# TomasDelaney/A-Deep-Reinforcement-Learning-Enabled-Soft-Exoskeleton-for-Parkinson-s-Patients

Measured on AMD Instinct MI355X. Metric: env steps/sec (batched exo sim) + TD7 grad-steps/sec at 1/2/4/8 MI355X, higher is better.
Workload: dtype f64 sim + bf16 TD7

## Files before the change

### a-deep-reinforcement-learning-enabled-soft-exoskeleton-for-parkinson-s-patients_amd/csrc/td7_fused.h

```cpp
#pragma once
#include <hip/hip_runtime.h>

#include <cstdint>

#include "exo_amd.h"
#include "philox.h"

namespace td7f {

typedef float floatx4 __attribute__((ext_vector_type(4)));
typedef __bf16 bf16x8 __attribute__((ext_vector_type(8)));
typedef _Float16 halfx8 __attribute__((ext_vector_type(8)));
typedef uint32_t u32x4 __attribute__((ext_vector_type(4)));
typedef uint32_t u32x2 __attribute__((ext_vector_type(2)));

template <typename T>
__device__ __forceinline__ T ldg(const T *p) {
    return *(const __attribute__((address_space(1))) T *)p;
}
template <typename T>
__device__ __forceinline__ void stg(T *p, T v) {
    *(__attribute__((address_space(1))) T *)p = v;
}

constexpr int NW = 4;
constexpr int NKG = 2;
constexpr int NTH = 64 * NW * NKG;
constexpr int PD = TD7F_PD;
constexpr int TR = 16;

enum Prec : int { PREC_BF16 = 1, PREC_F16 = 2, PREC_F32 = 3 };
enum Act : int { ACT_NONE = 0, ACT_RELU = 1, ACT_ELU = 2, ACT_TANH = 3 };

template <int P> struct Ty;
struct Ty16 {
    using E = uint16_t;
    static constexpr int EB = 2, KD = 32, SUB = 1;
};
template <> struct Ty<PREC_BF16> : Ty16 {
    static __device__ __forceinline__ floatx4 mfma(u32x4 a, u32x4 b, floatx4 c, int = 0) {
        return __builtin_amdgcn_mfma_f32_16x16x32_bf16(__builtin_bit_cast(bf16x8, a), __builtin_bit_cast(bf16x8, b),
                                                       c, 0, 0, 0);
    }
    static __device__ __forceinline__ uint16_t bits(float v) { return __builtin_bit_cast(uint16_t, (__bf16)v); }
    static __device__ __forceinline__ float val(uint16_t b) { return (float)__builtin_bit_cast(__bf16, b); }
    static constexpr float gs = 1.f;
};
template <> struct Ty<PREC_F16> : Ty16 {
    static __device__ __forceinline__ floatx4 mfma(u32x4 a, u32x4 b, floatx4 c, int = 0) {
        return __builtin_amdgcn_mfma_f32_16x16x32_f16(__builtin_bit_cast(halfx8, a), __builtin_bit_cast(halfx8, b), c,
                                                      0, 0, 0);
    }
    static __device__ __forceinline__ uint16_t bits(float v) { return __builtin_bit_cast(uint16_t, (_Float16)v); }
    static __device__ __forceinline__ float val(uint16_t b) { return (float)__builtin_bit_cast(_Float16, b); }
    static constexpr float gs = 1024.f;
};
template <> struct Ty<PREC_F32> {
    using E = float;
    static constexpr int EB = 4, KD = 16, SUB = 4;
    static __device__ __forceinline__ floatx4 mfma(u32x4 a, u32x4 b, floatx4 c, int j) {
        const floatx4 af = __builtin_bit_cast(floatx4, a), bf = __builtin_bit_cast(floatx4, b);
        return __builtin_amdgcn_mfma_f32_16x16x4f32(af[j], bf[j], c, 0, 0, 0);
    }
    static __device__ __forceinline__ float bits(float v) { return v; }
    static __device__ __forceinline__ float val(float b) { return b; }
    static constexpr float gs = 1.f;
};

__device__ __forceinline__ float act_fwd(int act, float x) {
    if (act == ACT_RELU) return x > 0.f ? x : 0.f;
    if (act == ACT_ELU) return x > 0.f ? x : __expf(x) - 1.0f;
    if (act == ACT_TANH) return tanhf(x);
    return x;
}
__device__ __forceinline__ float act_grad(int act, float y) {
    if (act == ACT_RELU) return y > 0.f ? 1.f : 0.f;
    if (act == ACT_ELU) return y > 0.f ? 1.f : y + 1.f;
    if (act == ACT_TANH) return 1.f - y * y;
    return 1.f;
}

struct Lin {
    const u32x4 *wf, *wb;
    const float *b;
    int N, K, ksf, ksb;
    const float *w;
    long ldw;
};

struct GDesc {
    const u32x4 *wp;
    int ks;
    int t0;
};

__device__ __forceinline__ void kgroup_range(int ks, int kg, int &kb, int &ke) {
    const int kA = ks >= 2 * PD ? ((ks / 2 + PD - 1) / PD) * PD : ks;
    kb = kg ? kA : 0;
    ke = kg ? ks : kA;
}

template <int TH>
__device__ __forceinline__ void ring_fill(u32x4 (&R)[PD][TH], const GDesc &g) {
    const int wv = threadIdx.x >> 6, w = wv % NW, kg = wv / NW, lane = threadIdx.x & 63;
    int kb, ke;
    kgroup_range(g.ks, kg, kb, ke);
    const bool live = ke > kb;
#pragma unroll
    for (int p = 0; p < PD; ++p)
#pragma unroll
        for (int i = 0; i < TH; ++i) {
            R[p][i] = ldg(g.wp + (live ? ((size_t)(g.t0 + w + NW * i) * g.ks + kb + p) * 64 : 0) + lane);
            __builtin_amdgcn_sched_barrier(0);
        }
}

struct EpiSrc {
    const float *p;
    long ld;
    int c0, row0, nrows, ncols;
};
template <int RT, int TH>
__device__ __forceinline__ void epi_prefetch(const EpiSrc &e, int t0, floatx4 (&ep)[RT][TH]) {
#pragma unroll
    for (int i = 0; i < TH; ++i) {
        const int wv = threadIdx.x >> 6;
        const int col = 16 * (t0 + wv % NW + NW * i) + 4 * ((threadIdx.x & 63) >> 4) - e.c0;
        const bool mine = (i < (TH + 1) / 2) == (wv < NW);
#pragma unroll
        for (int r = 0; r < RT; ++r) {
            const int row = (threadIdx.x & 15) + TR * r;
            const bool ok = e.p && mine && col >= 0 && col < e.ncols && (e.ld == 0 || e.row0 + row < e.nrows);
            ep[r][i] = ok ? ldg((const floatx4 *)(e.p + (e.ld ? (long)(e.row0 + row) * e.ld : 0) + col))
                          : floatx4{0.f, 0.f, 0.f, 0.f};
        }
    }
}

template <int P, int RT, int TH>
__device__ __forceinline__ void gemm(char *lds, int a_off, int lda, const GDesc &g, u32x4 (&R)[PD][TH],
                                     floatx4 (&acc)[RT][TH], const GDesc *next, const EpiSrc &es,
                                     floatx4 (&ep)[RT][TH]) {
    const int wv = threadIdx.x >> 6, w = wv % NW, kg = wv / NW, lane = threadIdx.x & 63;
    int kb, ke, nb = 0, ne = 0;
    kgroup_range(g.ks, kg, kb, ke);
    if (next) kgroup_range(next->ks, kg, nb, ne);
    epi_prefetch(es, g.t0, ep);
#pragma unroll
    for (int r = 0; r < RT; ++r)
#pragma unroll
        for (int i = 0; i < TH; ++i) acc[r][i] = floatx4{0.f, 0.f, 0.f, 0.f};
    if (ke > kb) {
        const u32x4 *bp[TH];
#pragma unroll
        for (int i = 0; i < TH; ++i) bp[i] = g.wp + ((size_t)(g.t0 + w + NW * i) * g.ks + kb) * 64 + lane;
        const char *ap = lds + a_off + ((lane & 15) * lda + 8 * (lane >> 4) + 32 * kb) * 2;
        const int n = ke - kb;
        u32x4 an[RT];
#pragma unroll
        for (int r = 0; r < RT; ++r) an[r] = *(const u32x4 *)(ap + r * TR * lda * 2);
        int s0 = 0;
        for (; s0 + PD < n; s0 += PD) {
#pragma unroll
            for (int p = 0; p < PD; ++p) {
                const int s = s0 + p;
                u32x4 x[RT];
#pragma unroll
                for (int r = 0; r < RT; ++r) {
                    x[r] = an[r];
                    an[r] = *(const u32x4 *)(ap + (r * TR * lda + 32 * (s + 1)) * 2);
                }
#pragma unroll
                for (int j = 0; j < Ty<P>::SUB; ++j)
#pragma unroll
                    for (int i = 0; i < TH; ++i) {
#pragma unroll
                        for (int r = 0; r < RT; ++r) acc[r][i] = Ty<P>::mfma(R[p][i], x[r], acc[r][i], j);
                        __builtin_amdgcn_sched_barrier(0);
                    }
#pragma unroll
                for (int i = 0; i < TH; ++i) {
                    R[p][i] = ldg(bp[i] + (s + PD) * 64);
                    __builtin_amdgcn_sched_barrier(0);
                }
            }
        }
        const u32x4 *np[TH];
        if (ne > nb)
#pragma unroll
            for (int i = 0; i < TH; ++i) np[i] = next->wp + ((size_t)(next->t0 + w + NW * i) * next->ks + nb) * 64 + lane;
#pragma unroll
        for (int p = 0; p < PD; ++p) {
            const int s = s0 + p;
            u32x4 x[RT];
#pragma unroll
            for (int r = 0; r < RT; ++r) {
                x[r] = an[r];
                if (p + 1 < PD) an[r] = *(const u32x4 *)(ap + (r * TR * lda + 32 * (s + 1)) * 2);
            }
#pragma unroll
            for (int j = 0; j < Ty<P>::SUB; ++j)
#pragma unroll
                for (int i = 0; i < TH; ++i) {
#pragma unroll
                    for (int r = 0; r < RT; ++r) acc[r][i] = Ty<P>::mfma(R[p][i], x[r], acc[r][i], j);
                    __builtin_amdgcn_sched_barrier(0);
                }
            if (ne > nb) {
#pragma unroll
                for (int i = 0; i < TH; ++i) {
                    R[p][i] = ldg(np[i] + p * 64);
                    __builtin_amdgcn_sched_barrier(0);
                }
            }
        }
    } else if (next) {
        ring_fill(R, *next);
    }
    constexpr int h = (TH + 1) / 2;
    floatx4 *red = (floatx4 *)lds + ((w * 64 + lane) * RT) * TH;
#pragma unroll
    for (int r = 0; r < RT; ++r)
#pragma unroll
        for (int i = 0; i < TH; ++i)
            if ((i < h) != (kg == 0)) red[r * TH + i] = acc[r][i];
    __syncthreads();
#pragma unroll
    for (int r = 0; r < RT; ++r)
#pragma unroll
        for (int i = 0; i < TH; ++i)
            if ((i < h) == (kg == 0)) acc[r][i] += red[r * TH + i];
}

constexpr int red_bytes(int rt, int tpw) { return NW * 64 * rt * tpw * 16; }

template <int TH>
__device__ __forceinline__ bool owns(int i) {
    return (i < (TH + 1) / 2) == ((threadIdx.x >> 6) < NW);
}
__device__ __forceinline__ int acc_col(int t0, int i) {
    const int wv = threadIdx.x >> 6;
    return 16 * (t0 + wv % NW + NW * i) + 4 * ((threadIdx.x & 63) >> 4);
}
__device__ __forceinline__ int acc_row(int r) { return (threadIdx.x & 15) + TR * r; }

struct R16 {
    int off, ld;
};
struct R32 {
    int off, ld;
};
constexpr R16 NO16{-1, 0};
constexpr R32 NO32{-1, 0};
__device__ __forceinline__ uint16_t *p16(char *lds, R16 r, int row, int col) {
    return (uint16_t *)(lds + r.off) + row * r.ld + col;
}
__device__ __forceinline__ float *p32(char *lds, R32 r, int row, int col) {
    return (float *)(lds + r.off) + row * r.ld + col;
}
template <int P>
__device__ __forceinline__ u32x2 pack4(const float (&v)[4]) {
    return u32x2{(uint32_t)Ty<P>::bits(v[0]) | ((uint32_t)Ty<P>::bits(v[1]) << 16),
                 (uint32_t)Ty<P>::bits(v[2]) | ((uint32_t)Ty<P>::bits(v[3]) << 16)};
}
template <int P>
__device__ __forceinline__ typename Ty<P>::E *pe(char *lds, R16 r, int row, int col) {
    return (typename Ty<P>::E *)(lds + r.off + row * r.ld * 2) + col;
}
template <int P>
__device__ __forceinline__ void put4(char *lds, R16 r, int row, int col, const float (&v)[4]) {
    if constexpr (Ty<P>::EB == 4) *(floatx4 *)pe<P>(lds, r, row, col) = floatx4{v[0], v[1], v[2], v[3]};
    else *(u32x2 *)pe<P>(lds, r, row, col) = pack4<P>(v);
}

template <int P, int RT, int TH>
__device__ __forceinline__ void epi_fwd(char *lds, const floatx4 (&acc)[RT][TH], const floatx4 (&bias)[RT][TH], int N,
                                        int act, R16 o16, int col0, R32 o32, float *g, long gld, int row0,
                                        int nrows) {
#pragma unroll
    for (int i = 0; i < TH; ++i) {
        if (!owns<TH>(i)) continue;
        const int n = acc_col(0, i);
        if (n >= N) continue;
        const floatx4 b = bias[0][i];
#pragma unroll
        for (int r = 0; r < RT; ++r) {
            const int row = acc_row(r);
            float v[4];
#pragma unroll
            for (int e = 0; e < 4; ++e) v[e] = act_fwd(act, acc[r][i][e] + b[e]);
            if (o16.off >= 0) put4<P>(lds, o16, row, col0 + n, v);
            if (o32.off >= 0) *(floatx4 *)p32(lds, o32, row, n) = floatx4{v[0], v[1], v[2], v[3]};
            if (g && row0 + row < nrows) stg((floatx4 *)(g + (long)(row0 + row) * gld + n), floatx4{v[0], v[1], v[2], v[3]});
        }
    }
}

template <int P, int RT, int TH>
__device__ __forceinline__ void epi_bwd(char *lds, const floatx4 (&acc)[RT][TH], int t0, int c0, int c1, int act,
                                        const floatx4 (&yv_)[RT][TH], R32 o32, float *g, long gld, R16 o16,
                                        float *part, int row0, int nrows) {
#pragma unroll
    for (int i = 0; i < TH; ++i) {
        if (!owns<TH>(i)) continue;
        const int col = acc_col(t0, i);
        const bool in = col >= c0 && col < c1;
        const int m = col - c0;
        float cs[4] = {0.f, 0.f, 0.f, 0.f};
#pragma unroll
        for (int r = 0; r < RT; ++r) {
            const int row = acc_row(r);
            const bool live = in && row0 + row < nrows;
            float v[4];
#pragma unroll
            for (int e = 0; e < 4; ++e) v[e] = live ? acc[r][i][e] * (1.f / Ty<P>::gs) : 0.f;
            if (live && act != ACT_NONE) {
                const floatx4 yv = yv_[r][i];
#pragma unroll
                for (int e = 0; e < 4; ++e) v[e] *= act_grad(act, yv[e]);
            }
#pragma unroll
            for (int e = 0; e < 4; ++e) cs[e] += v[e];
            if (in) {
                if (o32.off >= 0) *(floatx4 *)p32(lds, o32, row, m) = floatx4{v[0], v[1], v[2], v[3]};
                if (o16.off >= 0) {
                    float s[4] = {v[0] * Ty<P>::gs, v[1] * Ty<P>::gs, v[2] * Ty<P>::gs, v[3] * Ty<P>::gs};
                    put4<P>(lds, o16, row, m, s);
                }
                if (g && row0 + row < nrows) stg((floatx4 *)(g + (long)(row0 + row) * gld + m), floatx4{v[0], v[1], v[2], v[3]});
            }
        }
        if (part) {
#pragma unroll
            for (int e = 0; e < 4; ++e)
#pragma unroll
                for (int o = 1; o < 16; o <<= 1) cs[e] += __shfl_xor(cs[e], o, 64);
            if (in && (threadIdx.x & 15) == 0) stg((floatx4 *)(part + m), floatx4{cs[0], cs[1], cs[2], cs[3]});
        }
    }
}

template <int P, int NC>
__device__ __forceinline__ void thin(char *lds, R16 in, int xc0, int K, R32 wl, int ncols, R32 out, float scale) {
    constexpr int KS = NTH / TR;
    const int row = threadIdx.x / KS, sl = threadIdx.x % KS;
    float acc[NC];
#pragma unroll
    for (int j = 0; j < NC; ++j) acc[j] = 0.f;
#pragma unroll 2
    for (int k = sl; k < K; k += KS) {
        const float x = Ty<P>::val(*pe<P>(lds, in, row, xc0 + k));
#pragma unroll
        for (int j = 0; j < NC; ++j) acc[j] += x * *p32(lds, wl, j, k);
    }
#pragma unroll
    for (int j = 0; j < NC; ++j) {
#pragma unroll
        for (int o = KS / 2; o > 0; o >>= 1) acc[j] += __shfl_xor(acc[j], o, 64);
    }
    if (sl == 0)
#pragma unroll
        for (int j = 0; j < NC; ++j)
            if (j < ncols) *p32(lds, out, row, j) = acc[j] * scale;
}
constexpr int THIN_NC = 8;

template <int P>
__device__ __forceinline__ void make_dp(char *lds, R32 dy, int N, int act, const float *y, long yld, R16 o16,
                                        float *part, int row0, int nrows) {
    for (int n = threadIdx.x; n < N; n += NTH) {
        float cs = 0.f;
        for (int r = 0; r < TR; ++r) {
            float v = *p32(lds, dy, r, n);
            if (row0 + r >= nrows) v = 0.f;
            else if (act != ACT_NONE) v *= act_grad(act, ldg(y + (long)(row0 + r) * yld + n));
            *p32(lds, dy, r, n) = v;
            *pe<P>(lds, o16, r, n) = Ty<P>::bits(v * Ty<P>::gs);
            cs += v;
        }
        if (part) stg(part + n, cs);
    }
}

__device__ __forceinline__ void store_rows16(char *lds, R16 src, int col0, uint16_t *dst, long dld, int ncols,
                                             int rows, int row0, int nrows) {
    if (ncols % 8 == 0 && dld % 8 == 0 && col0 % 8 == 0 && src.ld % 8 == 0) {
        const int nq = ncols / 8;
        for (int k = threadIdx.x; k < rows * nq; k += NTH) {
            const int row = k / nq, c = 8 * (k - row * nq);
            if (row0 + row < nrows) stg((u32x4 *)(dst + (long)(row0 + row) * dld + c), *(const u32x4 *)p16(lds, src, row, col0 + c));
        }
        return;
    }
    for (int k = threadIdx.x; k < rows * ncols; k += NTH) {
        const int row = k / ncols, c = k - row * ncols;
        if (row0 + row < nrows) stg(dst + (long)(row0 + row) * dld + c, *p16(lds, src, row, col0 + c));
    }
}

struct RowStage {
    float v[TR];
};
__device__ __forceinline__ void row_issue(RowStage &s, const float *src, long sld, int ncols, int row0, int nrows) {
    const int c = min((int)threadIdx.x, ncols - 1);
#pragma unroll
    for (int r = 0; r < TR; ++r) s.v[r] = ldg(src + (long)(row0 + r < nrows ? row0 + r : row0) * sld + c);
}
__device__ __forceinline__ void row_add(RowStage &s, const RowStage &o) {
#pragma unroll
    for (int r = 0; r < TR; ++r) s.v[r] += o.v[r];
}
template <int P>
__device__ __forceinline__ void row_put16(char *lds, const RowStage &s, R16 dst, int col0, int ncols, int row0,
                                          int nrows, float scale = 1.f) {
    if ((int)threadIdx.x < ncols)
#pragma unroll
        for (int r = 0; r < TR; ++r)
            *pe<P>(lds, dst, r, col0 + threadIdx.x) = Ty<P>::bits(row0 + r < nrows ? s.v[r] * scale : 0.f);
}
__device__ __forceinline__ void row_put32(char *lds, const RowStage &s, R32 dst, int ncols, int row0, int nrows) {
    if ((int)threadIdx.x < ncols)
#pragma unroll
        for (int r = 0; r < TR; ++r) *p32(lds, dst, r, threadIdx.x) = row0 + r < nrows ? s.v[r] : 0.f;
}
struct Row16Stage {
    uint32_t v[TR];
};
__device__ __forceinline__ void row16_issue(Row16Stage &s, const uint16_t *src, long sld, int ncols, int row0,
                                            int nrows) {
    const int c = 2 * min((int)threadIdx.x, (ncols - 1) / 2);
#pragma unroll
    for (int r = 0; r < TR; ++r)
        s.v[r] = ldg((const uint32_t *)(src + (long)(row0 + r < nrows ? row0 + r : row0) * sld + c));
}
__device__ __forceinline__ void row16_put(char *lds, const Row16Stage &s, R16 dst, int col0, int ncols, int row0,
                                          int nrows) {
    const int c = 2 * threadIdx.x;
    if (c < ncols)
#pragma unroll
        for (int r = 0; r < TR; ++r) {
            const uint32_t v = row0 + r < nrows ? s.v[r] : 0u;
            *p16(lds, dst, r, col0 + c) = (uint16_t)(v & 0xffffu);
            if (c + 1 < ncols) *p16(lds, dst, r, col0 + c + 1) = (uint16_t)(v >> 16);
        }
}
template <int NC>
struct ThinStage {
    float v[NC];
};
template <int NC>
__device__ __forceinline__ void thin_issue(ThinStage<NC> &s, const float *W, long ldw, int j0, bool trans, int ncols,
                                           int K) {
    const int k = min((int)threadIdx.x, K - 1);
#pragma unroll
    for (int j = 0; j < NC; ++j) {
        const int jj = min(j, ncols - 1);
        s.v[j] = ldg(trans ? W + (long)k * ldw + j0 + jj : W + (long)(j0 + jj) * ldw + k);
    }
}
template <int P, int NC>
__device__ __forceinline__ void thin_put(char *lds, const ThinStage<NC> &s, R32 wl, int ncols, int K) {
    if ((int)threadIdx.x < K)
#pragma unroll
        for (int j = 0; j < NC; ++j) *p32(lds, wl, j, threadIdx.x) = j < ncols ? Ty<P>::val(Ty<P>::bits(s.v[j])) : 0.f;
}

__device__ __forceinline__ uint16_t *blk8(uint16_t *base, long ld, int c, int r) {
    return base + ((long)(c >> 4) * (ld >> 5) + (r >> 5)) * 512 + ((c & 15) + 16 * ((r & 31) >> 3)) * 8;
}
__device__ __forceinline__ float *blk4(float *base, long ld, int c, int r) {
    return base + ((long)(c >> 4) * (ld >> 4) + (r >> 4)) * 256 + ((c & 15) + 16 * ((r & 15) >> 2)) * 4;
}

template <int P>
__device__ __forceinline__ void save_xt(char *lds, R16 src, int col0, int ncols, void *xt_, long ld, int rows,
                                        int row0) {
    if constexpr (P == PREC_F32) {
        float *xt = (float *)xt_;
        for (int k = threadIdx.x; k < ncols * (rows / TR); k += NTH) {
            const int c = k % ncols, rb = (k / ncols) * TR;
            float v[TR];
#pragma unroll
            for (int j = 0; j < TR; ++j) v[j] = *pe<P>(lds, src, rb + j, col0 + c);
#pragma unroll
            for (int q = 0; q < 4; ++q)
                stg((floatx4 *)blk4(xt, ld, c, row0 + rb + 4 * q), floatx4{v[4 * q], v[4 * q + 1], v[4 * q + 2], v[4 * q + 3]});
        }
        return;
    }
    uint16_t *xt = (uint16_t *)xt_;
    if (col0 % 2 == 0 && src.ld % 2 == 0) {
        for (int k = threadIdx.x; k < ((ncols + 1) / 2) * (rows / TR); k += NTH) {
            const int c = 2 * (k % ((ncols + 1) / 2)), rb = (k / ((ncols + 1) / 2)) * TR;
            uint32_t lo[8], hi[8];
#pragma unroll
            for (int j = 0; j < 8; ++j) {
                const uint32_t r0 = *(const uint32_t *)p16(lds, src, rb + 2 * j, col0 + c);
                const uint32_t r1 = *(const uint32_t *)p16(lds, src, rb + 2 * j + 1, col0 + c);
                lo[j] = (r0 & 0xffffu) | (r1 << 16);
                hi[j] = (r0 >> 16) | (r1 & 0xffff0000u);
            }
            stg((u32x4 *)blk8(xt, ld, c, row0 + rb), u32x4{lo[0], lo[1], lo[2], lo[3]});
            stg((u32x4 *)blk8(xt, ld, c, row0 + rb + 8), u32x4{lo[4], lo[5], lo[6], lo[7]});
            if (c + 1 < ncols) {
                stg((u32x4 *)blk8(xt, ld, c + 1, row0 + rb), u32x4{hi[0], hi[1], hi[2], hi[3]});
                stg((u32x4 *)blk8(xt, ld, c + 1, row0 + rb + 8), u32x4{hi[4], hi[5], hi[6], hi[7]});
            }
        }
        return;
    }
    for (int k = threadIdx.x; k < ncols * (rows / TR); k += NTH) {
        const int c = k % ncols, rb = (k / ncols) * TR;
        uint32_t v[8];
#pragma unroll
        for (int j = 0; j < 8; ++j)
            v[j] = (uint32_t)*p16(lds, src, rb + 2 * j, col0 + c) |
                   ((uint32_t)*p16(lds, src, rb + 2 * j + 1, col0 + c) << 16);
        stg((u32x4 *)blk8(xt, ld, c, row0 + rb), u32x4{v[0], v[1], v[2], v[3]});
        stg((u32x4 *)blk8(xt, ld, c, row0 + rb + 8), u32x4{v[4], v[5], v[6], v[7]});
    }
}

template <int P>
__device__ __forceinline__ void norm_fwd(char *lds, R32 h, int N, int rows, float eps, R16 o16, int col0, R16 o16b,
                                         int col0b, R32 o32, float *g, long gld, float *mean_lds, float *gmean,
                                         int row0, int nrows) {
    const int tpr = NTH / rows;
    const int row = threadIdx.x / tpr, j0 = threadIdx.x % tpr;
    float acc = 0.f;
    for (int n = j0; n < N; n += tpr) acc += fabsf(*p32(lds, h, row, n));
    for (int o = tpr / 2; o > 0; o >>= 1) acc += __shfl_xor(acc, o, 64);
    const float m = acc / N, s = fmaxf(m, eps);
    for (int n = j0; n < N; n += tpr) {
        const float v = *p32(lds, h, row, n) / s;
        const auto b = Ty<P>::bits(v);
        if (o16.off >= 0) *pe<P>(lds, o16, row, col0 + n) = b;
        if (o16b.off >= 0) *pe<P>(lds, o16b, row, col0b + n) = b;
        if (o32.off >= 0) *p32(lds, o32, row, n) = v;
        if (g && row0 + row < nrows) stg(g + (long)(row0 + row) * gld + n, v);
    }
    if (j0 == 0) {
        if (mean_lds) mean_lds[row] = m;
        if (gmean && row0 + row < nrows) stg(gmean + row0 + row, m);
    }
}

template <int P>
__device__ __forceinline__ void norm_bwd(char *lds, R32 dy, R32 h, const float *mean, int N, float eps, float *dot,
                                         R16 o16, void *dpt, long dpt_ld, float *part, int row0, int nrows) {
    {
        constexpr int tpr = NTH / TR;
        const int row = threadIdx.x / tpr, j0 = threadIdx.x % tpr;
        float acc = 0.f;
        for (int n = j0; n < N; n += tpr) acc += *p32(lds, dy, row, n) * *p32(lds, h, row, n);
        for (int o = tpr / 2; o > 0; o >>= 1) acc += __shfl_xor(acc, o, 64);
        if (j0 == 0) dot[row] = acc;
    }
    __syncthreads();
    for (int n = threadIdx.x; n < N; n += NTH) {
        float csum = 0.f;
        uint32_t v[8];
        float f[TR];
#pragma unroll
        for (int r = 0; r < TR; ++r) {
            const float m = mean[r];
            float gx;
            if (m >= eps) {
                const float inv = 1.0f / m, c = dot[r] * inv * inv / N;
                const float xv = *p32(lds, h, r, n);
                const float sg = (xv > 0.f) ? 1.f : ((xv < 0.f) ? -1.f : 0.f);
                gx = *p32(lds, dy, r, n) * inv - sg * c;
            } else {
                gx = *p32(lds, dy, r, n) / eps;
            }
            if (row0 + r >= nrows) gx = 0.f;
            csum += gx;
            const auto hb = Ty<P>::bits(gx * Ty<P>::gs);
            *pe<P>(lds, o16, r, n) = hb;
            if constexpr (P == PREC_F32) {
                f[r] = hb;
            } else {
                if (r & 1) v[r >> 1] |= (uint32_t)hb << 16;
                else v[r >> 1] = hb;
            }
        }
        if (dpt) {
            if constexpr (P == PREC_F32) {
#pragma unroll
                for (int q = 0; q < 4; ++q)
                    stg((floatx4 *)blk4((float *)dpt, dpt_ld, n, row0 + 4 * q), floatx4{f[4 * q], f[4 * q + 1], f[4 * q + 2], f[4 * q + 3]});
            } else {
                stg((u32x4 *)blk8((uint16_t *)dpt, dpt_ld, n, row0), u32x4{v[0], v[1], v[2], v[3]});
                stg((u32x4 *)blk8((uint16_t *)dpt, dpt_ld, n, row0 + 8), u32x4{v[4], v[5], v[6], v[7]});
            }
        }
        if (part) stg(part + n, csum);
    }
}

struct Noise {
    uint64_t seed;
    uint32_t tag;
    unsigned long long *counter;
    uint32_t *ticket;
    float *sigma;
    float sigma_dec, clip, scale;
    const float *z;
    const int32_t *dec_count;
};

#ifdef EXO_STAMPS
static __device__ unsigned long long *g_td7f_stamps;
#define FSTAMP(si)                                                                                 \
    do {                                                                                           \
        unsigned long long _t;                                                                     \
        __builtin_amdgcn_sched_barrier(0);                                                         \
        asm volatile("s_memtime %0\n\ts_waitcnt lgkmcnt(0)" : "=s"(_t)::"memory");                \
        __builtin_amdgcn_sched_barrier(0);                                                         \
        if (g_td7f_stamps && threadIdx.x == 0 && (si) < 64)                                        \
            stg(g_td7f_stamps + (size_t)(blockIdx.x + blockIdx.y * gridDim.x) * 64 + (si), _t);    \
        ++(si);                                                                                    \
    } while (0)
#else
#define FSTAMP(si) do {} while (0)
#endif


template <int P, int RT, int TH>
__device__ __forceinline__ void layer_fwd(char *lds, u32x4 (&R)[PD][TH], R16 a, const Lin &L, const GDesc *next,
                                          int act, R16 o16, int col0, R32 o32, float *g, long gld, int row0,
                                          int nrows, int &si) {
    FSTAMP(si);
    floatx4 acc[RT][TH], bias[RT][TH];
    const GDesc gd{L.wf, L.ksf, 0};
    gemm<P, RT, TH>(lds, a.off, a.ld, gd, R, acc, next, EpiSrc{L.b, 0, 0, 0, 0, L.N}, bias);
    FSTAMP(si);
    epi_fwd<P, RT, TH>(lds, acc, bias, L.N, act, o16, col0, o32, g, gld, row0, nrows);
    __syncthreads();
}
template <int P, int RT, int TH>
__device__ __forceinline__ void layer_fwd(char *lds, u32x4 (&R)[PD][TH], R16 a, const Lin &L, const Lin *next, int act,
                                          R16 o16, int col0, R32 o32, float *g, long gld, int row0, int nrows,
                                          int &si) {
    GDesc gn{nullptr, 0, 0};
    if (next) gn = GDesc{next->wf, next->ksf, 0};
    layer_fwd<P, RT, TH>(lds, R, a, L, next ? &gn : (const GDesc *)nullptr, act, o16, col0, o32, g, gld, row0, nrows,
                         si);
}

template <int P, int NC>
__device__ __forceinline__ void layer_thin_fwd(char *lds, R16 a, const Lin &L, R32 wl, int act, R32 out, int rows,
                                               float *g, long gld, int row0, int nrows, int &si) {
    FSTAMP(si);
    thin<P, NC>(lds, a, 0, L.K, wl, L.N, out, 1.f);
    __syncthreads();
    for (int k = threadIdx.x; k < rows * L.N; k += NTH) {
        const int row = k / L.N, n = k - row * L.N;
        const float v = act_fwd(act, *p32(lds, out, row, n) + ldg(L.b + n));
        *p32(lds, out, row, n) = v;
        if (g && row0 + row < nrows) stg(g + (long)(row0 + row) * gld + n, v);
    }
    __syncthreads();
}

__device__ __forceinline__ void zero_lds(char *lds, int bytes) {
    for (int i = threadIdx.x * 16; i < bytes; i += NTH * 16) *(u32x4 *)(lds + i) = u32x4{0u, 0u, 0u, 0u};
}

template <int P>
__device__ __forceinline__ void noise_rows(char *lds, R32 a, int A, int rows, int row0, int nrows, const Noise &nz,
                                           float *out, R16 o1, int c1, R16 o2, int c2, bool ticket = true) {
    const float sg = ldg(nz.sigma);
    const unsigned long long call = ldg(nz.counter);
    for (int k = threadIdx.x; k < rows * A; k += NTH) {
        const int row = k / A, c = k - row * A;
        float v = 0.f;
        if (row0 + row < nrows) {
            const uint32_t i = (uint32_t)((row0 + row) * A + c);
            float z;
            if (nz.z) {
                z = ldg(nz.z + i);
            } else {
                uint32_t r[4];
                philox_block(nz.seed, nz.tag, call, i >> 1, r);
                float z0, z1;
                box_muller(r, z0, z1);
                z = (i & 1) ? z1 : z0;
            }
            float e = z * sg;
            if (nz.clip > 0.f) e = fminf(fmaxf(e, -nz.clip), nz.clip);
            v = fminf(fmaxf(*p32(lds, a, row, c) + e, -1.0f), 1.0f) * nz.scale;
            if (out) stg(out + i, v);
        }
        const auto b = Ty<P>::bits(v);
        if (o1.off >= 0) *pe<P>(lds, o1, row, c1 + c) = b;
        if (o2.off >= 0) *pe<P>(lds, o2, row, c2 + c) = b;
    }
    __syncthreads();
    if (ticket && threadIdx.x == 0) {
        __threadfence();
        if (atomicAdd(nz.ticket, 1u) == gridDim.x * gridDim.y - 1) {
            *nz.sigma = sg - (nz.dec_count ? nz.sigma_dec * (float)*nz.dec_count : nz.sigma_dec);
            if (!nz.z) *nz.counter = call + 1ull;
            *nz.ticket = 0u;
        }
    }
}

inline int round_up(int x, int m) { return (x + m - 1) / m * m; }
inline int kd_of(int prec) { return prec == PREC_F32 ? 16 : 32; }
inline int ks_of(int k, int kd = 32) { return round_up((k + kd - 1) / kd, PD); }
inline int ld16(int n, int kd = 32) { return ks_of(n, kd) * 32 + 16; }

struct Bump {
    int off;
    explicit Bump(int rt) : off(red_bytes(rt, 5)) {}
    R16 r16(int rows, int ld) {
        R16 r{off, ld};
        off += round_up(rows * ld * 2, 16);
        return r;
    }
    R32 r32(int rows, int ld) {
        R32 r{off, ld};
        off += round_up(rows * ld * 4, 16);
        return r;
    }
};

inline Lin lin_of(const td7f_lin &l) {
    return Lin{(const u32x4 *)l.wf, (const u32x4 *)l.wb, l.b, l.n_out, l.n_in, l.ksf, l.ksb, l.w, (long)l.ldw};
}
inline Noise noise_of(const td7f_noise &n) {
    return Noise{n.seed, n.tag, n.counter, n.ticket, n.sigma, n.sigma_dec, n.clip, n.scale, n.z, n.dec_count};
}

inline int th_of(const td7f_lin *ls, int n) {
    int th = 0;
    for (int i = 0; i < n; ++i) {
        if (!ls[i].wf || ls[i].ksf <= 0 || ls[i].ksf % PD || !ls[i].b) return -1;
        if (ls[i].n_out <= 16) {
            if (!ls[i].w || ls[i].ldw < ls[i].n_in) return -1;
            continue;
        }
        if (ls[i].n_out % 4) return -1;
        const int t = round_up((ls[i].n_out + 15) / 16, NW) / NW;
        if (th && t != th) return -1;
        th = t;
    }
    return th ? th : 4;
}

constexpr int LDS_MAX = 160 * 1024;

extern thread_local bool td7f_probe_mode;

template <typename K, typename A>
int launch(K kernel, dim3 grid, int lds, A args, hipStream_t st) {
    if (lds > LDS_MAX) return EXO_EINVAL;
    if (td7f_probe_mode) return EXO_OK;
    if (hipFuncSetAttribute((const void *)kernel, hipFuncAttributeMaxDynamicSharedMemorySize, lds) != hipSuccess)
        return EXO_EDEVICE;
    hipLaunchKernelGGL(kernel, grid, dim3(NTH), lds, st, args);
    return hipGetLastError() == hipSuccess ? EXO_OK : EXO_EDEVICE;
}

#define DISPATCH(PREC, TH, KERNEL, ...)                                                                 \
    ((PREC) == PREC_BF16  ? ((TH) == 5 ? launch(KERNEL<PREC_BF16, 5>, __VA_ARGS__)                      \
                                       : launch(KERNEL<PREC_BF16, 4>, __VA_ARGS__))                     \
     : (PREC) == PREC_F16 ? ((TH) == 5 ? launch(KERNEL<PREC_F16, 5>, __VA_ARGS__)                       \
                                       : launch(KERNEL<PREC_F16, 4>, __VA_ARGS__))                      \
                          : ((TH) == 5 ? launch(KERNEL<PREC_F32, 5>, __VA_ARGS__)                       \
                                       : launch(KERNEL<PREC_F32, 4>, __VA_ARGS__)))

}
```

### a-deep-reinforcement-learning-enabled-soft-exoskeleton-for-parkinson-s-patients_amd/csrc/td7_fused.hip

```cpp
#include "td7_fused.h"

#include <algorithm>
#include <cstdlib>

#include "adam_math.h"
#include "philox.h"

namespace td7f {

struct PackJob {
    const float *w;
    long ld;
    int N, K;
    u32x4 *wf, *wb;
    int ksf, ntf, ksb, ntb;
};
struct PackArgs {
    int njobs;
    long start[TD7F_MAX_PACK + 1];
    PackJob j[TD7F_MAX_PACK];
};

template <int P>
__device__ __forceinline__ float w_at(const PackJob &J, int n, int c) {
    const bool ok = n < J.N && c < J.K;
    const float x = ldg(J.w + (long)(ok ? n : 0) * J.ld + (ok ? c : 0));
    return ok ? x : 0.f;
}
__device__ __forceinline__ void pack_item_f32(const PackJob &J, long k, long nf, bool vec) {
    const int l = (int)(k & 63);
    float x[4];
    u32x4 *dst;
    if (k < nf) {
        const long blk = k >> 6;
        const int t = (int)(blk / J.ksf), s = (int)(blk % J.ksf);
        const int n = 16 * t + (l & 15), k0 = 16 * s + 4 * (l >> 4);
        if (vec && n < J.N && k0 + 4 <= J.K) {
            const floatx4 a0 = ldg((const floatx4 *)(J.w + (long)n * J.ld + k0));
            x[0] = a0[0], x[1] = a0[1], x[2] = a0[2], x[3] = a0[3];
        } else {
#pragma unroll
            for (int j = 0; j < 4; ++j) x[j] = w_at<PREC_F32>(J, n, k0 + j);
        }
        dst = J.wf + k;
    } else {
        const long blk = (k - nf) >> 6;
        const int t = (int)(blk / J.ksb), s = (int)(blk % J.ksb);
        const int c = 16 * t + (l & 15), n0 = 16 * s + 4 * (l >> 4);
#pragma unroll
        for (int j = 0; j < 4; ++j) x[j] = w_at<PREC_F32>(J, n0 + j, c);
        dst = J.wb + (k - nf);
    }
    stg(dst, __builtin_bit_cast(u32x4, floatx4{x[0], x[1], x[2], x[3]}));
}

template <int P>
__global__ __launch_bounds__(256) void pack_kernel(PackArgs a) {
    const PackJob J = a.j[blockIdx.y];
    if constexpr (P == PREC_F32) {
        const long nf = (long)J.ntf * J.ksf * 64, total = nf + (long)J.ntb * J.ksb * 64;
        const bool vec = (J.ld % 4) == 0 && (reinterpret_cast<uintptr_t>(J.w) & 15) == 0;
        for (long k = (long)blockIdx.x * 256 + threadIdx.x; k < total; k += (long)gridDim.x * 256)
            pack_item_f32(J, k, nf, vec);
        return;
    }
    const long nf = (long)J.ntf * J.ksf * 64, total = nf + (long)J.ntb * J.ksb * 64;
    const bool vec = (J.ld % 4) == 0 && (reinterpret_cast<uintptr_t>(J.w) & 15) == 0;
    for (long k = (long)blockIdx.x * 256 + threadIdx.x; k < total; k += (long)gridDim.x * 256) {
        const int l = (int)(k & 63);
        float x[8];
        u32x4 *dst;
        if (k < nf) {
            const long blk = k >> 6;
            const int t = (int)(blk / J.ksf), s = (int)(blk % J.ksf);
            const int n = 16 * t + (l & 15), k0 = 32 * s + 8 * (l >> 4);
            if (vec && n < J.N && k0 + 8 <= J.K) {
                const floatx4 a0 = ldg((const floatx4 *)(J.w + (long)n * J.ld + k0));
                const floatx4 a1 = ldg((const floatx4 *)(J.w + (long)n * J.ld + k0 + 4));
                x[0] = a0[0], x[1] = a0[1], x[2] = a0[2], x[3] = a0[3];
                x[4] = a1[0], x[5] = a1[1], x[6] = a1[2], x[7] = a1[3];
            } else {
#pragma unroll
                for (int j = 0; j < 8; ++j) x[j] = w_at<P>(J, n, k0 + j);
            }
            dst = J.wf + k;
        } else {
            const long blk = (k - nf) >> 6;
            const int t = (int)(blk / J.ksb), s = (int)(blk % J.ksb);
            const int c = 16 * t + (l & 15), n0 = 32 * s + 8 * (l >> 4);
#pragma unroll
            for (int j = 0; j < 8; ++j) x[j] = w_at<P>(J, n0 + j, c);
            dst = J.wb + (k - nf);
        }
        uint32_t v[4];
#pragma unroll
        for (int jj = 0; jj < 4; ++jj)
            v[jj] = (uint32_t)Ty<P>::bits(x[2 * jj]) | ((uint32_t)Ty<P>::bits(x[2 * jj + 1]) << 16);
        stg(dst, u32x4{v[0], v[1], v[2], v[3]});
    }
}

struct APOpt {
    float *p, *m, *v, *step;
    float lr, b1, b2, eps, wd;
};
struct APSeg {
    const float *g;
    long off;
    int n, opt;
};
struct APJob {
    float *p, *m, *v;
    const float *g;
    u32x4 *wf, *wb;
    int opt, N, K, nch, ksf, ksb, vec;
};
struct AdamPackArgs {
    APOpt o[TD7_ADAM_MAX_OPT];
    APSeg s[TD7_ADAM_MAX_SEG];
    int q0[TD7_ADAM_MAX_SEG + 1];
    APJob j[TD7F_MAX_ADAM_PACK];
    int jb[TD7F_MAX_ADAM_PACK + 1];
    int nopt, nseg, njobs;
    uint32_t *ticket;
};

template <int P>
__global__ __launch_bounds__(256) void adam_pack_kernel(AdamPackArgs a) {
    __shared__ float coef[TD7_ADAM_MAX_OPT][2];
    __shared__ u32x4 tt[32][8];
    if ((int)threadIdx.x < a.nopt) {
        const APOpt o = a.o[threadIdx.x];
        const float t = *o.step + 1.0f;
        coef[threadIdx.x][0] = o.lr / (1.0f - powf(o.b1, t));
        coef[threadIdx.x][1] = sqrtf(1.0f - powf(o.b2, t));
    }
    __syncthreads();
    const int b = blockIdx.x;
    if (b < a.jb[a.njobs]) {
        int q = 0;
        while (q + 1 < a.njobs && b >= a.jb[q + 1]) ++q;
        const APJob &J = a.j[q];
        const APOpt &o = a.o[J.opt];
        const float ss = coef[J.opt][0], bc = coef[J.opt][1];
        const int i = (b - a.jb[q]) * 256 + threadIdx.x;
        const int tile = i >> 3, r = i & 7;
        const int G = tile / J.nch, c0 = 8 * (tile - G * J.nch);
        const int n0 = 8 * G, n = n0 + r;
        const bool rv = n < J.N;
        float x[8];
#pragma unroll
        for (int jj = 0; jj < 8; ++jj) x[jj] = 0.f;
        if (rv) {
            const long e = (long)n * J.K + c0;
            const int ne = min(8, J.K - c0);
            float pp[8], mm[8], vv[8], gg[8];
            if (J.vec) {
#pragma unroll
                for (int h = 0; h < 2; ++h) {
                    const long eh = e + (h < ne / 4 ? 4 * h : 0);
                    const floatx4 p4 = ldg((const floatx4 *)(J.p + eh)), m4 = ldg((const floatx4 *)(J.m + eh));
                    const floatx4 v4 = ldg((const floatx4 *)(J.v + eh)), g4 = ldg((const floatx4 *)(J.g + eh));
#pragma unroll
                    for (int u = 0; u < 4; ++u)
                        pp[4 * h + u] = p4[u], mm[4 * h + u] = m4[u], vv[4 * h + u] = v4[u], gg[4 * h + u] = g4[u];
                }
            } else {
#pragma unroll
                for (int jj = 0; jj < 8; ++jj) {
                    const long ej = e + (jj < ne ? jj : 0);
                    pp[jj] = ldg(J.p + ej), mm[jj] = ldg(J.m + ej), vv[jj] = ldg(J.v + ej), gg[jj] = ldg(J.g + ej);
                }
            }
#pragma unroll
            for (int jj = 0; jj < 8; ++jj) adam_one(pp[jj], gg[jj], mm[jj], vv[jj], ss, bc, o.b1, o.b2, o.eps, o.wd, 1.0f);
            if (J.vec) {
#pragma unroll
                for (int h = 0; h < 2; ++h)
                    if (h < ne / 4) {
                        stg((floatx4 *)(J.p + e + 4 * h), floatx4{pp[4 * h], pp[4 * h + 1], pp[4 * h + 2], pp[4 * h + 3]});
                        stg((floatx4 *)(J.m + e + 4 * h), floatx4{mm[4 * h], mm[4 * h + 1], mm[4 * h + 2], mm[4 * h + 3]});
                        stg((floatx4 *)(J.v + e + 4 * h), floatx4{vv[4 * h], vv[4 * h + 1], vv[4 * h + 2], vv[4 * h + 3]});
                    }
            } else {
#pragma unroll
                for (int jj = 0; jj < 8; ++jj)
                    if (jj < ne) stg(J.p + e + jj, pp[jj]), stg(J.m + e + jj, mm[jj]), stg(J.v + e + jj, vv[jj]);
            }
#pragma unroll
            for (int jj = 0; jj < 8; ++jj) x[jj] = jj < ne ? pp[jj] : 0.f;
        }
        if constexpr (P == PREC_F32) {
            __shared__ float tf[32][8][8];
            if (rv)
#pragma unroll
                for (int h = 0; h < 2; ++h) {
                    const int c = c0 + 4 * h;
                    stg(J.wf + ((long)(n >> 4) * J.ksf + (c >> 4)) * 64 + (n & 15) + 16 * ((c & 15) >> 2),
                        __builtin_bit_cast(u32x4, floatx4{x[4 * h], x[4 * h + 1], x[4 * h + 2], x[4 * h + 3]}));
                }
            const int slot = threadIdx.x >> 3;
#pragma unroll
            for (int jj = 0; jj < 8; ++jj) tf[slot][r][jj] = x[jj];
            __syncthreads();
            const int c = c0 + r;
            if (J.wb && n0 < J.N && c < J.K)
#pragma unroll
                for (int h = 0; h < 2; ++h) {
                    const int nn = n0 + 4 * h;
                    stg(J.wb + ((long)(c >> 4) * J.ksb + (nn >> 4)) * 64 + (c & 15) + 16 * ((nn & 15) >> 2),
                        __builtin_bit_cast(u32x4, floatx4{tf[slot][4 * h][r], tf[slot][4 * h + 1][r],
                                                          tf[slot][4 * h + 2][r], tf[slot][4 * h + 3][r]}));
                }
        } else {
        uint32_t w[4];
#pragma unroll
        for (int jj = 0; jj < 4; ++jj)
            w[jj] = (uint32_t)Ty<P>::bits(x[2 * jj]) | ((uint32_t)Ty<P>::bits(x[2 * jj + 1]) << 16);
        if (rv)
            stg(J.wf + ((long)(n >> 4) * J.ksf + (c0 >> 5)) * 64 + (n & 15) + 16 * ((c0 & 31) >> 3),
                u32x4{w[0], w[1], w[2], w[3]});
        const int slot = threadIdx.x >> 3;
        tt[slot][r] = u32x4{w[0], w[1], w[2], w[3]};
        __syncthreads();
        const int c = c0 + r;
        if (J.wb && n0 < J.N && c < J.K) {
            const uint16_t *T = reinterpret_cast<const uint16_t *>(&tt[slot][0]);
            uint32_t d[4];
#pragma unroll
            for (int jj = 0; jj < 4; ++jj) d[jj] = (uint32_t)T[16 * jj + r] | ((uint32_t)T[16 * jj + 8 + r] << 16);
            stg(J.wb + ((long)(c >> 4) * J.ksb + (n0 >> 5)) * 64 + (c & 15) + 16 * ((n0 & 31) >> 3),
                u32x4{d[0], d[1], d[2], d[3]});
        }
        }
    } else if (a.nseg > 0) {
        const int pb = b - a.jb[a.njobs], npb = gridDim.x - a.jb[a.njobs];
        for (int gi = pb * 256 + threadIdx.x; gi < a.q0[a.nseg]; gi += npb * 256) {
            int lo = 0, hi = a.nseg - 1;
            while (lo < hi) {
                const int mid = (lo + hi + 1) >> 1;
                if (gi >= a.q0[mid]) lo = mid;
                else hi = mid - 1;
            }
            const APSeg sg = a.s[lo];
            const APOpt o = a.o[sg.opt];
            const float ss = coef[sg.opt][0], bc = coef[sg.opt][1];
            const long e0 = 4L * (gi - a.q0[lo]);
            const int ne = (int)min(4L, (long)sg.n - e0);
            float *p = o.p + sg.off + e0, *m = o.m + sg.off + e0, *v = o.v + sg.off + e0;
            const float *g = sg.g + e0;
            for (int e = 0; e < ne; ++e) adam_one(p[e], g[e], m[e], v[e], ss, bc, o.b1, o.b2, o.eps, o.wd, 1.0f);
        }
    }
    __syncthreads();
    if (threadIdx.x == 0) {
        const uint32_t done = atomicAdd(a.ticket, 1u);
        if (done == gridDim.x - 1) {
            for (int k = 0; k < a.nopt; ++k) *a.o[k].step = *a.o[k].step + 1.0f;
            *a.ticket = 0u;
        }
    }
}

struct SelectArgs {
    Lin zs[3], ac[4];
    int act_enc, act_actor;
    const float *obs;
    int n, S, A, Z, Ha;
    float *out;
    Noise nz;
    R16 X, H1, H2, CAT;
    R32 F, TW, FT;
    int lds_bytes;
    int tile0, ticket;
    void *zimg;
};

#define RING_START(first)      \
    u32x4 R[PD][TH];           \
    ring_fill(R, GDesc{(first).wf, (first).ksf, 0})

__device__ __forceinline__ R16 rows_of(R16 r, int t) { return R16{r.off + t * TR * r.ld * 2, r.ld}; }
__device__ __forceinline__ R32 rows_of(R32 r, int t) { return R32{r.off + t * TR * r.ld * 4, r.ld}; }

template <int P, int TH, int RT, int ZM = 0>
__global__ __launch_bounds__(NTH) void select_kernel(SelectArgs a) {
    extern __shared__ __attribute__((aligned(16))) char lds[];
    constexpr int rows = RT * TR;
    int row0;
    if constexpr (RT == 1) row0 = (a.tile0 + blockIdx.x) * rows;
    else row0 = blockIdx.x * rows;
    int si = 0;
    FSTAMP(si);
    RowStage so[RT];
    ThinStage<THIN_NC> tw;
    using E = typename Ty<P>::E;
    static_assert(RT * TR * (int)sizeof(E) <= 64, "ZM 2 staging: 16 rows x 512 words at most");
#pragma unroll
    for (int t = 0; t < RT; ++t) row_issue(so[t], a.obs, a.S, a.S, row0 + t * TR, a.n);
    if constexpr (ZM != 1) thin_issue(tw, a.ac[3].w, a.ac[3].ldw, 0, false, a.A, a.ac[3].K);
    const int zw = a.Z * (int)sizeof(E) / 4;
    constexpr int ZPT = ZM == 2 ? (16 * 512 + NTH - 1) / NTH : 1;
    uint32_t zv[ZPT];
    if constexpr (ZM == 2) {
        const uint32_t *zi = (const uint32_t *)a.zimg;
#pragma unroll
        for (int u = 0; u < ZPT; ++u) {
            const int k = threadIdx.x + u * NTH, r = k / zw, c = k - r * zw;
            zv[u] = (r < rows && row0 + r < a.n) ? zi[(long)(row0 + r) * zw + c] : 0u;
        }
    }
    RING_START(ZM == 2 ? a.ac[0] : a.zs[0]);
    zero_lds(lds, a.lds_bytes);
    __syncthreads();
#pragma unroll
    for (int t = 0; t < RT; ++t) row_put16<P>(lds, so[t], rows_of(a.X, t), 0, a.S, row0 + t * TR, a.n);
    if constexpr (ZM != 1) thin_put<P>(lds, tw, a.TW, a.A, a.ac[3].K);
    if constexpr (ZM == 2) {
#pragma unroll
        for (int u = 0; u < ZPT; ++u) {
            const int k = threadIdx.x + u * NTH, r = k / zw, c = k - r * zw;
            if (r < rows) *(uint32_t *)(pe<P>(lds, a.CAT, r, a.Ha) + c * (4 / (int)sizeof(E))) = zv[u];
        }
    }
    __syncthreads();
    if constexpr (ZM != 2) {
        layer_fwd<P, RT, TH>(lds, R, a.X, a.zs[0], &a.zs[1], a.act_enc, a.H1, 0, NO32, nullptr, 0, row0, a.n, si);
        layer_fwd<P, RT, TH>(lds, R, a.H1, a.zs[1], &a.zs[2], a.act_enc, a.H2, 0, NO32, nullptr, 0, row0, a.n, si);
        layer_fwd<P, RT, TH>(lds, R, a.H2, a.zs[2], ZM == 1 ? (const Lin *)nullptr : &a.ac[0], ACT_NONE, NO16, 0, a.F,
                             nullptr, 0, row0, a.n, si);
        norm_fwd<P>(lds, a.F, a.Z, rows, 1e-8f, a.CAT, a.Ha, NO16, 0, NO32, nullptr, 0, nullptr, nullptr, row0, a.n);
        __syncthreads();
    }
    if constexpr (ZM == 1) {
        uint32_t *zo = (uint32_t *)a.zimg;
        for (int k = threadIdx.x; k < rows * zw; k += NTH) {
            const int r = k / zw, c = k - r * zw;
            if (row0 + r < a.n)
                zo[(long)(row0 + r) * zw + c] = *(const uint32_t *)(pe<P>(lds, a.CAT, r, a.Ha) + c * (4 / (int)sizeof(E)));
        }
        return;
    }
    layer_fwd<P, RT, TH>(lds, R, a.X, a.ac[0], &a.ac[1], ACT_NONE, NO16, 0, a.F, nullptr, 0, row0, a.n, si);
    norm_fwd<P>(lds, a.F, a.Ha, rows, 1e-8f, a.CAT, 0, NO16, 0, NO32, nullptr, 0, nullptr, nullptr, row0, a.n);
    __syncthreads();
    if (a.F.off == a.H1.off) zero_lds(lds + a.H1.off, a.H2.off + rows * a.H2.ld * 2 - a.H1.off);
    layer_fwd<P, RT, TH>(lds, R, a.CAT, a.ac[1], &a.ac[2], a.act_actor, a.H1, 0, NO32, nullptr, 0, row0, a.n, si);
    layer_fwd<P, RT, TH>(lds, R, a.H1, a.ac[2], (const Lin *)nullptr, a.act_actor, a.H2, 0, NO32, nullptr, 0, row0, a.n, si);
    if constexpr (RT == 1) {
        layer_thin_fwd<P, THIN_NC>(lds, a.H2, a.ac[3], a.TW, ACT_TANH, a.FT, rows, nullptr, 0, row0, a.n, si);
    } else {
        FSTAMP(si);
#pragma unroll
        for (int t = 0; t < RT; ++t)
            thin<P, THIN_NC>(lds, rows_of(a.H2, t), 0, a.ac[3].K, a.TW, a.A, rows_of(a.FT, t), 1.f);
        __syncthreads();
        for (int k = threadIdx.x; k < rows * a.A; k += NTH) {
            const int row = k / a.A, c = k - row * a.A;
            *p32(lds, a.FT, row, c) = act_fwd(ACT_TANH, *p32(lds, a.FT, row, c) + ldg(a.ac[3].b + c));
        }
        __syncthreads();
    }
    if constexpr (RT == 1) noise_rows<P>(lds, a.FT, a.A, rows, row0, a.n, a.nz, a.out, NO16, 0, NO16, 0, a.ticket != 0);
    else noise_rows<P>(lds, a.FT, a.A, rows, row0, a.n, a.nz, a.out, NO16, 0, NO16, 0);
}

struct TargetArgs {
    Lin enc[6], ac[4], cr[8];
    int act_enc, act_actor, act_critic;
    const float *ns;
    int B, S, A, Z, Ha, Hc;
    Noise nz;
    void *img;
    float *qt;
    R16 X, H1, H2, CATA, CATZ, OUT, CAT;
    R32 F, TW;
    int lds_a, lds_b;
};

template <int P, int TH>
__global__ __launch_bounds__(NTH) void target_a_kernel(TargetArgs a) {
    extern __shared__ __attribute__((aligned(16))) char lds[];
    constexpr int RT = 1, rows = TR;
    const int row0 = blockIdx.x * rows, B = a.B, Z = a.Z;
    int si = 0;
    FSTAMP(si);
    RowStage sn;
    ThinStage<THIN_NC> tw;
    row_issue(sn, a.ns, a.S, a.S, row0, B);
    thin_issue(tw, a.ac[3].w, a.ac[3].ldw, 0, false, a.A, a.ac[3].K);
    RING_START(a.enc[0]);
    zero_lds(lds, a.lds_a);
    __syncthreads();
    row_put16<P>(lds, sn, a.X, 0, a.S, row0, B);
    thin_put<P>(lds, tw, a.TW, a.A, a.ac[3].K);
    __syncthreads();
    layer_fwd<P, RT, TH>(lds, R, a.X, a.enc[0], &a.enc[1], a.act_enc, a.H1, 0, NO32, nullptr, 0, row0, B, si);
    layer_fwd<P, RT, TH>(lds, R, a.H1, a.enc[1], &a.enc[2], a.act_enc, a.H2, 0, NO32, nullptr, 0, row0, B, si);
    layer_fwd<P, RT, TH>(lds, R, a.H2, a.enc[2], &a.ac[0], ACT_NONE, NO16, 0, a.F, nullptr, 0, row0, B, si);
    norm_fwd<P>(lds, a.F, Z, rows, 1e-8f, a.CATA, a.Ha, a.CATZ, 0, NO32, nullptr, 0, nullptr, nullptr, row0, B);
    __syncthreads();
    layer_fwd<P, RT, TH>(lds, R, a.X, a.ac[0], &a.ac[1], ACT_NONE, NO16, 0, a.F, nullptr, 0, row0, B, si);
    norm_fwd<P>(lds, a.F, a.Ha, rows, 1e-8f, a.CATA, 0, NO16, 0, NO32, nullptr, 0, nullptr, nullptr, row0, B);
    __syncthreads();
    layer_fwd<P, RT, TH>(lds, R, a.CATA, a.ac[1], &a.ac[2], a.act_actor, a.H1, 0, NO32, nullptr, 0, row0, B, si);
    layer_fwd<P, RT, TH>(lds, R, a.H1, a.ac[2], &a.enc[3], a.act_actor, a.H2, 0, NO32, nullptr, 0, row0, B, si);
    layer_thin_fwd<P, THIN_NC>(lds, a.H2, a.ac[3], a.TW, ACT_TANH, a.F, rows, nullptr, 0, row0, B, si);
    noise_rows<P>(lds, a.F, a.A, rows, row0, B, a.nz, nullptr, a.CATZ, Z, a.OUT, 2 * Z);
    __syncthreads();
    layer_fwd<P, RT, TH>(lds, R, a.CATZ, a.enc[3], &a.enc[4], a.act_enc, a.H1, 0, NO32, nullptr, 0, row0, B, si);
    layer_fwd<P, RT, TH>(lds, R, a.H1, a.enc[4], &a.enc[5], a.act_enc, a.H2, 0, NO32, nullptr, 0, row0, B, si);
    layer_fwd<P, RT, TH>(lds, R, a.H2, a.enc[5], (const Lin *)nullptr, ACT_NONE, a.OUT, 0, NO32, nullptr, 0, row0, B, si);
    for (int k = threadIdx.x; k < rows * Z; k += NTH) {
        const int row = k / Z, c = k - row * Z;
        *pe<P>(lds, a.OUT, row, Z + c) = *pe<P>(lds, a.CATZ, row, c);
    }
    __syncthreads();
    constexpr int EH = Ty<P>::EB / 2;
    const int ild = (2 * Z + a.A + 7) / 8 * 8 * EH;
    store_rows16(lds, a.OUT, 0, (uint16_t *)a.img, ild, ild, rows, row0, B);
}

template <int P, int TH>
__global__ __launch_bounds__(NTH) void target_b_kernel(TargetArgs a) {
    extern __shared__ __attribute__((aligned(16))) char lds[];
    constexpr int RT = 1, rows = TR;
    const int row0 = blockIdx.x * rows, B = a.B, Z = a.Z, h = blockIdx.y;
    const long ild = (2 * Z + a.A + 7) / 8 * 8;
    const Lin *cr = a.cr + h;
    int si = 0;
    FSTAMP(si);
    RowStage sn;
    ThinStage<1> tw;
    row_issue(sn, a.ns, a.S, a.S, row0, B);
    [[maybe_unused]] RowStage fa, fz0, fz1;
    [[maybe_unused]] Row16Stage sa, sc;
    if constexpr (P == PREC_F32) {
        const float *img = (const float *)a.img;
        row_issue(fa, img + 2 * Z, ild, a.A, row0, B);
        row_issue(fz0, img, ild, Z, row0, B);
        row_issue(fz1, img + Z, ild, Z, row0, B);
    } else {
        const uint16_t *img = (const uint16_t *)a.img;
        row16_issue(sa, img + 2 * Z, ild, a.A, row0, B);
        row16_issue(sc, img, ild, 2 * Z, row0, B);
    }
    thin_issue(tw, cr[6].w, cr[6].ldw, 0, false, 1, cr[6].K);
    RING_START(cr[0]);
    zero_lds(lds, a.lds_b);
    __syncthreads();
    row_put16<P>(lds, sn, a.X, 0, a.S, row0, B);
    if constexpr (P == PREC_F32) {
        row_put16<P>(lds, fa, a.X, a.S, a.A, row0, B);
        row_put16<P>(lds, fz0, a.CAT, a.Hc, Z, row0, B);
        row_put16<P>(lds, fz1, a.CAT, a.Hc + Z, Z, row0, B);
    } else {
        row16_put(lds, sa, a.X, a.S, a.A, row0, B);
        row16_put(lds, sc, a.CAT, a.Hc, 2 * Z, row0, B);
    }
    thin_put<P>(lds, tw, a.TW, 1, cr[6].K);
    __syncthreads();
    layer_fwd<P, RT, TH>(lds, R, a.X, cr[0], &cr[2], ACT_NONE, NO16, 0, a.F, nullptr, 0, row0, B, si);
    norm_fwd<P>(lds, a.F, a.Hc, rows, 1e-8f, a.CAT, 0, NO16, 0, NO32, nullptr, 0, nullptr, nullptr, row0, B);
    __syncthreads();
    layer_fwd<P, RT, TH>(lds, R, a.CAT, cr[2], &cr[4], a.act_critic, a.H1, 0, NO32, nullptr, 0, row0, B, si);
    layer_fwd<P, RT, TH>(lds, R, a.H1, cr[4], (const Lin *)nullptr, a.act_critic, a.H2, 0, NO32, nullptr, 0, row0, B, si);
    layer_thin_fwd<P, 1>(lds, a.H2, cr[6], a.TW, ACT_NONE, a.F, rows, a.qt + h, 2, row0, B, si);
}

struct FixedArgs {
    Lin enc[6];
    int act_enc;
    const float *s, *act;
    int B, S, A, Z;
    float *zs, *zsa;
    R16 X, H1, H2, CATZ;
    R32 F;
    int lds_bytes;
};

template <int P, int TH>
__global__ __launch_bounds__(NTH) void fixed_kernel(FixedArgs a) {
    extern __shared__ __attribute__((aligned(16))) char lds[];
    constexpr int RT = 1, rows = TR;
    const int row0 = blockIdx.x * rows, B = a.B, Z = a.Z;
    int si = 0;
    FSTAMP(si);
    RowStage ss, sa;
    row_issue(ss, a.s, a.S, a.S, row0, B);
    row_issue(sa, a.act, a.A, a.A, row0, B);
    RING_START(a.enc[0]);
    zero_lds(lds, a.lds_bytes);
    __syncthreads();
    row_put16<P>(lds, ss, a.X, 0, a.S, row0, B);
    row_put16<P>(lds, sa, a.CATZ, Z, a.A, row0, B);
    __syncthreads();
    layer_fwd<P, RT, TH>(lds, R, a.X, a.enc[0], &a.enc[1], a.act_enc, a.H1, 0, NO32, nullptr, 0, row0, B, si);
    layer_fwd<P, RT, TH>(lds, R, a.H1, a.enc[1], &a.enc[2], a.act_enc, a.H2, 0, NO32, nullptr, 0, row0, B, si);
    layer_fwd<P, RT, TH>(lds, R, a.H2, a.enc[2], &a.enc[3], ACT_NONE, NO16, 0, a.F, nullptr, 0, row0, B, si);
    norm_fwd<P>(lds, a.F, Z, rows, 1e-8f, a.CATZ, 0, NO16, 0, NO32, a.zs, Z, nullptr, nullptr, row0, B);
    __syncthreads();
    layer_fwd<P, RT, TH>(lds, R, a.CATZ, a.enc[3], &a.enc[4], a.act_enc, a.H1, 0, NO32, nullptr, 0, row0, B, si);
    layer_fwd<P, RT, TH>(lds, R, a.H1, a.enc[4], &a.enc[5], a.act_enc, a.H2, 0, NO32, nullptr, 0, row0, B, si);
    layer_fwd<P, RT, TH>(lds, R, a.H2, a.enc[5], (const Lin *)nullptr, ACT_NONE, NO16, 0, NO32, a.zsa, Z, row0, B, si);
}

thread_local bool td7f_probe_mode = false;
}

using namespace td7f;

static bool prec_ok(int p) { return p == PREC_BF16 || p == PREC_F16 || p == PREC_F32; }

extern "C" {

#ifdef EXO_STAMPS
int td7f_debug_set_stamps(unsigned long long *buf) {
    return hipMemcpyToSymbol(HIP_SYMBOL(g_td7f_stamps), &buf, sizeof(buf)) == hipSuccess ? 0 : -5;
}
#endif

int td7f_pack(int32_t prec, int32_t njobs, const td7f_pack_job *jobs, void *stream) {
    if (!prec_ok(prec) || njobs <= 0 || njobs > TD7F_MAX_PACK || !jobs) return EXO_EINVAL;
    const int kd = kd_of(prec);
    PackArgs a{};
    a.njobs = njobs;
    a.start[0] = 0;
    for (int q = 0; q < njobs; ++q) {
        const td7f_pack_job &J = jobs[q];
        if (!J.w || !J.wf || J.n_out <= 0 || J.n_in <= 0 || J.ld < J.n_in || J.ksf * kd < J.n_in ||
            J.ntf * 16 < J.n_out || (J.wb && (J.ksb * kd < J.n_out || J.ntb * 16 < J.n_in)))
            return EXO_EINVAL;
        a.j[q] = PackJob{J.w, (long)J.ld, J.n_out, J.n_in, (u32x4 *)J.wf, (u32x4 *)J.wb, J.ksf, J.ntf,
                         J.wb ? J.ksb : 0, J.wb ? J.ntb : 0};
        a.start[q + 1] = a.start[q] + (long)J.ntf * J.ksf * 64 + (J.wb ? (long)J.ntb * J.ksb * 64 : 0);
    }
    long most = 0;
    for (int q = 0; q < njobs; ++q) most = std::max(most, a.start[q + 1] - a.start[q]);
    const dim3 grid((unsigned)std::min<long>(1024, (most + 255) / 256), (unsigned)njobs);
    if (prec == PREC_BF16)
        hipLaunchKernelGGL(pack_kernel<PREC_BF16>, grid, dim3(256), 0, (hipStream_t)stream, a);
    else if (prec == PREC_F16)
        hipLaunchKernelGGL(pack_kernel<PREC_F16>, grid, dim3(256), 0, (hipStream_t)stream, a);
    else
        hipLaunchKernelGGL(pack_kernel<PREC_F32>, grid, dim3(256), 0, (hipStream_t)stream, a);
    return hipGetLastError() == hipSuccess ? EXO_OK : EXO_EDEVICE;
}

int td7f_adam_pack(int32_t prec, int32_t nopt, float *const *p, float *const *m, float *const *v, float *const *step,
                   const float *lr, const float *beta1, const float *beta2, const float *eps,
                   const float *weight_decay, int32_t nseg, const float *const *g, const int64_t *off, const int32_t *n,
                   const int32_t *opt, int32_t njobs, const td7f_pack_job *jobs, const int32_t *job_seg,
                   uint32_t *ticket, void *stream) {
    if (!prec_ok(prec) || nopt <= 0 || nopt > TD7_ADAM_MAX_OPT || nseg <= 0 ||
        nseg > TD7_ADAM_MAX_SEG || njobs < 0 || njobs > TD7F_MAX_ADAM_PACK || (njobs && (!jobs || !job_seg)) ||
        !ticket)
        return EXO_EINVAL;
    const int kd = kd_of(prec);
    AdamPackArgs a{};
    a.nopt = nopt;
    a.ticket = ticket;
    for (int k = 0; k < nopt; ++k) {
        if (!p[k] || !m[k] || !v[k] || !step[k]) return EXO_EINVAL;
        a.o[k] = APOpt{p[k], m[k], v[k], step[k], lr[k], beta1[k], beta2[k], eps[k], weight_decay[k]};
    }
    for (int k = 0; k < nseg; ++k)
        if (!g[k] || n[k] <= 0 || off[k] < 0 || opt[k] < 0 || opt[k] >= nopt) return EXO_EINVAL;
    long covered[TD7_ADAM_MAX_SEG] = {};
    a.jb[0] = 0;
    for (int q = 0; q < njobs; ++q) {
        const td7f_pack_job &J = jobs[q];
        const int k = job_seg[q];
        if (k < 0 || k >= nseg || !J.w || !J.wf || J.n_out <= 0 || J.n_in <= 0 || J.ld != J.n_in ||
            J.ksf * kd < J.n_in || J.ntf * 16 < J.n_out || (J.wb && (J.ksb * kd < J.n_out || J.ntb * 16 < J.n_in)))
            return EXO_EINVAL;
        const int o = opt[k];
        const long e = (long)(J.w - p[o]), sz = (long)J.n_out * J.n_in;
        if (e < off[k] || e + sz > off[k] + n[k]) return EXO_EINVAL;
        covered[k] += sz;
        const float *gq = g[k] + (e - off[k]);
        const bool vec = J.n_in % 4 == 0 &&
                         ((reinterpret_cast<uintptr_t>(J.w) | reinterpret_cast<uintptr_t>(m[o] + e) |
                           reinterpret_cast<uintptr_t>(v[o] + e) | reinterpret_cast<uintptr_t>(gq)) & 15) == 0;
        const int nch = (J.n_in + 7) / 8;
        a.j[q] = APJob{p[o] + e, m[o] + e, v[o] + e, gq, (u32x4 *)J.wf, (u32x4 *)J.wb, o, J.n_out, J.n_in, nch,
                       J.ksf, J.wb ? J.ksb : 0, vec ? 1 : 0};
        const long threads = (long)(J.n_out + 7) / 8 * nch * 8;
        a.jb[q + 1] = a.jb[q] + (int)((threads + 255) / 256);
    }
    a.njobs = njobs;
    long groups = 0;
    for (int k = 0; k < nseg; ++k) {
        if (covered[k] == n[k]) continue;
        if (covered[k] != 0) return EXO_EINVAL;
        a.s[a.nseg] = APSeg{g[k], (long)off[k], n[k], opt[k]};
        a.q0[a.nseg++] = (int)groups;
        groups += (n[k] + 3) / 4;
    }
    if (groups >= (1L << 30)) return EXO_ERANGE;
    a.q0[a.nseg] = (int)groups;
    const long plain = std::min<long>(64, (groups + 255) / 256);
    const unsigned grid = (unsigned)(a.jb[njobs] + plain);
    if (grid == 0) return EXO_OK;
    if (prec == PREC_BF16)
        hipLaunchKernelGGL(adam_pack_kernel<PREC_BF16>, dim3(grid), dim3(256), 0, (hipStream_t)stream, a);
    else if (prec == PREC_F16)
        hipLaunchKernelGGL(adam_pack_kernel<PREC_F16>, dim3(grid), dim3(256), 0, (hipStream_t)stream, a);
    else
        hipLaunchKernelGGL(adam_pack_kernel<PREC_F32>, dim3(grid), dim3(256), 0, (hipStream_t)stream, a);
    return hipGetLastError() == hipSuccess ? EXO_OK : EXO_EDEVICE;
}

int td7f_probe(int32_t on) {
    td7f::td7f_probe_mode = on != 0;
    return EXO_OK;
}

}

namespace {
template <int ZM>
int select_one(int prec, int th, int RT, dim3 g, int lds, const SelectArgs &a, hipStream_t st) {
    using namespace td7f;
    if (prec == PREC_F32)
        return th == 5 ? launch(select_kernel<PREC_F32, 5, 1, ZM>, g, lds, a, st)
                       : launch(select_kernel<PREC_F32, 4, 1, ZM>, g, lds, a, st);
    if (RT == 2)
        return prec == PREC_BF16 ? (th == 5 ? launch(select_kernel<PREC_BF16, 5, 2, ZM>, g, lds, a, st)
                                            : launch(select_kernel<PREC_BF16, 4, 2, ZM>, g, lds, a, st))
                                 : (th == 5 ? launch(select_kernel<PREC_F16, 5, 2, ZM>, g, lds, a, st)
                                            : launch(select_kernel<PREC_F16, 4, 2, ZM>, g, lds, a, st));
    return prec == PREC_BF16 ? (th == 5 ? launch(select_kernel<PREC_BF16, 5, 1, ZM>, g, lds, a, st)
                                        : launch(select_kernel<PREC_BF16, 4, 1, ZM>, g, lds, a, st))
                             : (th == 5 ? launch(select_kernel<PREC_F16, 5, 1, ZM>, g, lds, a, st)
                                        : launch(select_kernel<PREC_F16, 4, 1, ZM>, g, lds, a, st));
}
int select_mode(int zm, int prec, int th, int RT, dim3 g, int lds, const SelectArgs &a, hipStream_t st) {
    return zm == 1 ? select_one<1>(prec, th, RT, g, lds, a, st)
         : zm == 2 ? select_one<2>(prec, th, RT, g, lds, a, st)
                   : select_one<0>(prec, th, RT, g, lds, a, st);
}

int select_impl(int32_t prec, const int32_t *act, const td7f_lin *enc, const td7f_lin *actor, const float *obs,
                int32_t n, const td7f_noise *noise, float *out, int32_t wg_cap, int32_t rt, void *zimg, int zm,
                void *stream) {
    if (!prec_ok(prec) || !act || !enc || !actor || !obs || n <= 0 || wg_cap < 0 || rt < 0 || rt > 2 || zm < 0 ||
        zm > 2 || (zm != 1 && (!noise || !out)) || (zm != 0 && !zimg))
        return EXO_EINVAL;
    const int kd = kd_of(prec);
    td7f_lin all[7] = {enc[0], enc[1], enc[2], actor[0], actor[1], actor[2], actor[3]};
    const int th = th_of(all, 7);
    if (th != 4 && th != 5) return EXO_EINVAL;
    SelectArgs a{};
    for (int i = 0; i < 3; ++i) a.zs[i] = lin_of(enc[i]);
    for (int i = 0; i < 4; ++i) a.ac[i] = lin_of(actor[i]);
    a.act_enc = act[0];
    a.act_actor = act[1];
    a.obs = obs;
    a.n = n;
    a.S = enc[0].n_in;
    a.A = actor[3].n_out;
    a.Z = enc[2].n_out;
    a.Ha = actor[0].n_out;
    if (actor[0].n_in != a.S || actor[1].n_in != a.Ha + a.Z || a.A > THIN_NC || a.S > NTH) return EXO_EINVAL;
    a.out = out;
    if (zm != 1) a.nz = noise_of(*noise);
    a.zimg = zimg;
    if (zm != 0 && (((long)a.Z * (prec == PREC_F32 ? 4 : 2)) % 4 || ((long)a.Ha * (prec == PREC_F32 ? 4 : 2)) % 4 || a.Z > 512))
        return EXO_EINVAL;
    const char *rt_env = getenv("EXO_SELECT_RT");
    const int RT = prec == PREC_F32 ? 1
                   : rt_env && (rt_env[0] == '1' || rt_env[0] == '2') ? rt_env[0] - '0'
                   : rt ? rt : (n > 8192 ? 2 : 1);
    const int rows = RT * TR, hmax = std::max(enc[0].n_out, std::max(enc[1].n_out, std::max(a.Ha, actor[1].n_out)));
    Bump b(RT);
    a.X = b.r16(rows, ld16(a.S, kd));
    a.H1 = b.r16(rows, ld16(hmax, kd));
    a.H2 = b.r16(rows, ld16(hmax, kd));
    const int fld = std::max(std::max(a.Z, a.Ha), 16);
    if (rows * fld * 4 <= a.H2.off + rows * a.H2.ld * 2 - a.H1.off) {
        a.F = R32{a.H1.off, fld};
    } else {
        a.F = b.r32(rows, fld);
    }
    a.CAT = b.r16(rows, ld16(a.Ha + a.Z, kd));
    a.TW = b.r32(THIN_NC, actor[3].n_in);
    a.FT = b.r32(rows, 16);
    a.lds_bytes = b.off;
    const char *cap_env = getenv("EXO_SELECT_WG_CAP");
    const int ntiles = (n + rows - 1) / rows;
    const int cap = cap_env ? atoi(cap_env) : wg_cap;
    const hipStream_t st = (hipStream_t)stream;
    if (RT == 1 && cap > 0 && cap < ntiles) {
        for (int t0 = 0; t0 < ntiles; t0 += cap) {
            a.tile0 = t0;
            a.ticket = t0 + cap >= ntiles;
            const dim3 g(std::min(cap, ntiles - t0));
            const int rc = select_mode(zm, prec, th, 1, g, b.off, a, st);
            if (rc != EXO_OK) return rc;
        }
        return EXO_OK;
    }
    a.tile0 = 0;
    a.ticket = 1;
    return select_mode(zm, prec, th, RT, dim3(ntiles), b.off, a, st);
}
}

extern "C" {

int td7f_select(int32_t prec, const int32_t *act, const td7f_lin *enc, const td7f_lin *actor, const float *obs,
                int32_t n, const td7f_noise *noise, float *out, int32_t wg_cap, int32_t rt, void *stream) {
    return select_impl(prec, act, enc, actor, obs, n, noise, out, wg_cap, rt, nullptr, 0, stream);
}

int td7f_select_part(int32_t prec, const int32_t *act, const td7f_lin *enc, const td7f_lin *actor, const float *obs,
                     int32_t n, const td7f_noise *noise, float *out, int32_t wg_cap, int32_t rt, void *zimg,
                     int32_t mode, void *stream) {
    if (mode != 1 && mode != 2) return EXO_EINVAL;
    return select_impl(prec, act, enc, actor, obs, n, noise, out, wg_cap, rt, zimg, mode, stream);
}

int td7f_target(int32_t prec, const int32_t *act, const td7f_lin *tenc, const td7f_lin *tactor,
                const td7f_lin *tcritic, const float *ns, int32_t B, const td7f_noise *noise, void *img,
                float *qt, void *stream) {
    if (!prec_ok(prec) || !act || !tenc || !tactor || !tcritic || !ns || !noise || !img || !qt || B <= 0)
        return EXO_EINVAL;
    const int kd = kd_of(prec), eh = prec == PREC_F32 ? 2 : 1;
    td7f_lin all[18];
    for (int i = 0; i < 6; ++i) all[i] = tenc[i];
    for (int i = 0; i < 4; ++i) all[6 + i] = tactor[i];
    for (int i = 0; i < 8; ++i) all[10 + i] = tcritic[i];
    const int th = th_of(all, 18);
    if (th != 4 && th != 5) return EXO_EINVAL;
    TargetArgs a{};
    for (int i = 0; i < 6; ++i) a.enc[i] = lin_of(tenc[i]);
    for (int i = 0; i < 4; ++i) a.ac[i] = lin_of(tactor[i]);
    for (int i = 0; i < 8; ++i) a.cr[i] = lin_of(tcritic[i]);
    a.act_enc = act[0];
    a.act_actor = act[1];
    a.act_critic = act[2];
    a.ns = ns;
    a.B = B;
    a.S = tenc[0].n_in;
    a.A = tactor[3].n_out;
    a.Z = tenc[2].n_out;
    a.Ha = tactor[0].n_out;
    a.Hc = tcritic[0].n_out;
    if (tcritic[0].n_in != a.S + a.A || tcritic[2].n_in != a.Hc + 2 * a.Z || tcritic[4].n_in != a.Hc ||
        tenc[3].n_in != a.Z + a.A || a.A > THIN_NC || a.S > NTH)
        return EXO_EINVAL;
    a.nz = noise_of(*noise);
    a.img = img;
    a.qt = qt;
    const int rows = TR;
    int hmax = 0;
    for (int i = 0; i < 18; ++i) hmax = std::max(hmax, all[i].n_out);
    const int old = eh * round_up(2 * a.Z + a.A, 8);
    const int fld = std::max(hmax, 16);
    const bool wide_out = prec == PREC_F32 && old > ld16(a.Ha + a.Z, kd);
    Bump ba(1);
    a.X = ba.r16(rows, ld16(a.S + a.A, kd));
    if (wide_out) a.CATA = ba.r16(rows, ld16(a.Ha + a.Z, kd));
    a.H1 = ba.r16(rows, ld16(hmax, kd));
    a.H2 = ba.r16(rows, ld16(hmax, kd));
    if (!wide_out) a.CATA = ba.r16(rows, ld16(a.Ha + a.Z, kd));
    a.CATZ = ba.r16(rows, ld16(a.Z + a.A, kd));
    if (prec == PREC_F32) {
        if (!wide_out) a.OUT = R16{a.CATA.off, old};
        else if (rows * old * 2 <= a.CATA.off + rows * a.CATA.ld * 2 - a.X.off) a.OUT = R16{a.X.off, old};
        else a.OUT = ba.r16(rows, old);
        a.F = rows * fld * 4 <= a.H2.off + rows * a.H2.ld * 2 - a.H1.off ? R32{a.H1.off, fld} : ba.r32(rows, fld);
    } else {
        a.OUT = ba.r16(rows, old);
        a.F = ba.r32(rows, fld);
    }
    a.TW = ba.r32(THIN_NC, tactor[3].n_in);
    a.lds_a = ba.off;
    Bump bb(1);
    const R16 Xb = bb.r16(rows, ld16(a.S + a.A, kd)), H1b = bb.r16(rows, ld16(hmax, kd)), H2b = bb.r16(rows, ld16(hmax, kd));
    const R16 CATb = bb.r16(rows, ld16(a.Hc + 2 * a.Z, kd));
    const R32 Fb = bb.r32(rows, std::max(hmax, 16));
    const R32 TWb = bb.r32(1, tcritic[6].n_in);
    a.lds_b = bb.off;
    const hipStream_t st = (hipStream_t)stream;
    int rc = DISPATCH(prec, th, target_a_kernel, dim3((B + rows - 1) / rows), ba.off, a, st);
    if (rc != EXO_OK) return rc;
    TargetArgs b2 = a;
    b2.X = Xb;
    b2.H1 = H1b;
    b2.H2 = H2b;
    b2.CAT = CATb;
    b2.F = Fb;
    b2.TW = TWb;
    return DISPATCH(prec, th, target_b_kernel, dim3((B + rows - 1) / rows, 2), bb.off, b2, st);
}

int td7f_fixed(int32_t prec, const int32_t *act, const td7f_lin *fenc, const float *s, const float *action,
               int32_t B, float *zs, float *zsa, void *stream) {
    if (!prec_ok(prec) || !act || !fenc || !s || !action || !zs || !zsa || B <= 0) return EXO_EINVAL;
    const int kd = kd_of(prec);
    const int th = th_of(fenc, 6);
    if (th != 4 && th != 5) return EXO_EINVAL;
    FixedArgs a{};
    for (int i = 0; i < 6; ++i) a.enc[i] = lin_of(fenc[i]);
    a.act_enc = act[0];
    a.s = s;
    a.act = action;
    a.B = B;
    a.S = fenc[0].n_in;
    a.Z = fenc[2].n_out;
    a.A = fenc[3].n_in - a.Z;
    if (a.A <= 0 || a.A > THIN_NC || a.S > NTH) return EXO_EINVAL;
    a.zs = zs;
    a.zsa = zsa;
    const int rows = TR;
    int hmax = 0;
    for (int i = 0; i < 6; ++i) hmax = std::max(hmax, fenc[i].n_out);
    Bump b(1);
    a.X = b.r16(rows, ld16(a.S, kd));
    a.H1 = b.r16(rows, ld16(hmax, kd));
    a.H2 = b.r16(rows, ld16(hmax, kd));
    a.CATZ = b.r16(rows, ld16(a.Z + a.A, kd));
    a.F = b.r32(rows, std::max(hmax, 16));
    a.lds_bytes = b.off;
    return DISPATCH(prec, th, fixed_kernel, dim3((B + rows - 1) / rows), b.off, a, (hipStream_t)stream);
}

}
```

### a-deep-reinforcement-learning-enabled-soft-exoskeleton-for-parkinson-s-patients_amd/csrc/td7_fused_train.hip

```cpp
#include "td7_fused.h"
#include "td7_xcd_map.h"
#include "adam_math.h"

#include <algorithm>

namespace td7f {

struct XT {
    void *x;
    void *dp;
    float *part;
};

template <int P, int TH>
__device__ __forceinline__ void layer_bwd(char *lds, u32x4 (&R)[PD][TH], R16 a, const Lin &L, int c0, int c1,
                                          const GDesc *next, int act, const float *y, long yld, R32 o32, float *g,
                                          long gld, R16 o16, float *part, int row0, int nrows, int &si) {
    FSTAMP(si);
    floatx4 acc[1][TH], yv[1][TH];
    const GDesc gd{L.wb, L.ksb, c0 / 16};
    gemm<P, 1, TH>(lds, a.off, a.ld, gd, R, acc, next,
                   EpiSrc{act != ACT_NONE ? y : nullptr, yld, c0, row0, nrows, c1 - c0}, yv);
    FSTAMP(si);
    epi_bwd<P, 1, TH>(lds, acc, c0 / 16, c0, c1, act, yv, o32, g, gld, o16, part, row0, nrows);
    __syncthreads();
}

__device__ __forceinline__ GDesc fwd_of(const Lin &L) { return GDesc{L.wf, L.ksf, 0}; }
__device__ __forceinline__ GDesc bwd_of(const Lin &L, int c0) { return GDesc{L.wb, L.ksb, c0 / 16}; }

__device__ __forceinline__ void atomic_max_f(float *a, float v) {
    if (v >= 0.f) atomicMax((int *)a, __float_as_int(v));
    else atomicMin((unsigned int *)a, __float_as_uint(v));
}
__device__ __forceinline__ void atomic_min_f(float *a, float v) {
    if (v >= 0.f) atomicMin((int *)a, __float_as_int(v));
    else atomicMax((unsigned int *)a, __float_as_uint(v));
}

struct CriticArgs {
    Lin cr[8];
    int act;
    const float *s, *a, *zs, *zsa, *qt, *reward, *not_done;
    float discount, inv_b;
    const float *lo, *hi;
    float *run_max, *run_min;
    int B, S, A, Z, Hc;
    float *td, *q;
    float *y1, *y2;
    XT xt[8];
    long ld;
    R16 X, CAT, H1, H2, DP0, DP1;
    R32 H0, DY, F, TW;
    int small_off;
    int lds_bytes;
    int phase;
    float *qs, *h0s, *ms;
};

template <int P, int TH>
__global__ __launch_bounds__(NTH) void critic_kernel(CriticArgs a) {
    extern __shared__ __attribute__((aligned(16))) char lds[];
    const int row0 = blockIdx.x * TR, B = a.B, h = blockIdx.y, Hc = a.Hc, Z = a.Z, tile = blockIdx.x;
    const Lin *cr = a.cr + h;
    const XT *xt = a.xt + h;
    float *mean = (float *)(lds + a.small_off), *dot = mean + TR;
    float *y1 = a.y1 + (long)h * B * Hc, *y2 = a.y2 + (long)h * B * Hc;
    int si = 0;
    FSTAMP(si);
    u32x4 R[PD][TH];
    const long Bp = (long)gridDim.x * TR;
    if (a.phase == 2) {
        constexpr int PER = TR * 320 / NTH;
        const float *h0 = a.h0s + ((long)h * Bp + row0) * Hc;
        float v[PER];
#pragma unroll
        for (int j = 0; j < PER; ++j) {
            const int i = threadIdx.x + j * NTH;
            v[j] = i < TR * Hc ? ldg(h0 + i) : 0.f;
        }
        const float qv = threadIdx.x < TR ? ldg(a.qs + h * Bp + row0 + threadIdx.x) : 0.f;
        const float mv = threadIdx.x < TR ? ldg(a.ms + h * Bp + row0 + threadIdx.x) : 0.f;
        ring_fill(R, bwd_of(cr[6], 0));
        zero_lds(lds, a.lds_bytes);
        __syncthreads();
#pragma unroll
        for (int j = 0; j < PER; ++j) {
            const int i = threadIdx.x + j * NTH;
            if (i < TR * Hc) *p32(lds, a.H0, i / Hc, i % Hc) = v[j];
        }
        if (threadIdx.x < TR) {
            *p32(lds, a.F, threadIdx.x, 0) = qv;
            mean[threadIdx.x] = mv;
        }
        __syncthreads();
    } else {
    RowStage ss, sa, sz, szs;
    ThinStage<1> tw;
    row_issue(ss, a.s, a.S, a.S, row0, B);
    row_issue(sa, a.a, a.A, a.A, row0, B);
    row_issue(sz, a.zsa, Z, Z, row0, B);
    row_issue(szs, a.zs, Z, Z, row0, B);
    thin_issue(tw, cr[6].w, cr[6].ldw, 0, false, 1, cr[6].K);
    ring_fill(R, fwd_of(cr[0]));
    zero_lds(lds, a.lds_bytes);
    __syncthreads();
    row_put16<P>(lds, ss, a.X, 0, a.S, row0, B);
    row_put16<P>(lds, sa, a.X, a.S, a.A, row0, B);
    row_put16<P>(lds, sz, a.CAT, Hc, Z, row0, B);
    row_put16<P>(lds, szs, a.CAT, Hc + Z, Z, row0, B);
    thin_put<P>(lds, tw, a.TW, 1, cr[6].K);
    __syncthreads();
    layer_fwd<P, 1, TH>(lds, R, a.X, cr[0], &cr[2], ACT_NONE, NO16, 0, a.H0, nullptr, 0, row0, B, si);
    norm_fwd<P>(lds, a.H0, Hc, TR, 1e-8f, a.CAT, 0, NO16, 0, NO32, nullptr, 0, mean, nullptr, row0, B);
    __syncthreads();
    save_xt<P>(lds, a.X, 0, a.S + a.A, xt[0].x, a.ld, TR, row0);
    save_xt<P>(lds, a.CAT, 0, Hc + 2 * Z, xt[2].x, a.ld, TR, row0);
    layer_fwd<P, 1, TH>(lds, R, a.CAT, cr[2], &cr[4], a.act, a.H1, 0, NO32, y1, Hc, row0, B, si);
    const GDesc b3 = bwd_of(cr[6], 0);
    layer_fwd<P, 1, TH>(lds, R, a.H1, cr[4], &b3, a.act, a.H2, 0, NO32, y2, Hc, row0, B, si);
    save_xt<P>(lds, a.H1, 0, Hc, xt[4].x, a.ld, TR, row0);
    save_xt<P>(lds, a.H2, 0, Hc, xt[6].x, a.ld, TR, row0);
    layer_thin_fwd<P, 1>(lds, a.H2, cr[6], a.TW, ACT_NONE, a.F, TR, nullptr, 0, row0, B, si);
    if (a.phase == 1) {
        __syncthreads();
        float *h0 = a.h0s + ((long)h * Bp + row0) * Hc;
        for (int i = threadIdx.x; i < TR * Hc; i += NTH) stg(h0 + i, *p32(lds, a.H0, i / Hc, i % Hc));
        if (threadIdx.x < TR) {
            stg(a.qs + h * Bp + row0 + threadIdx.x, *p32(lds, a.F, threadIdx.x, 0));
            stg(a.ms + h * Bp + row0 + threadIdx.x, mean[threadIdx.x]);
        }
        return;
    }
    }
    if (threadIdx.x < TR) {
        const int r = threadIdx.x, b = row0 + r;
        float dq = 0.f;
        if (b < B) {
            const float qv = *p32(lds, a.F, r, 0);
            const float qm = fminf(ldg(a.qt + 2 * b), ldg(a.qt + 2 * b + 1));
            const float c = fminf(fmaxf(qm, ldg(a.lo)), ldg(a.hi));
            const float t = ldg(a.reward + b) + (ldg(a.not_done + b) * a.discount) * c;
            if (h == 0) {
                atomic_max_f(a.run_max, t);
                atomic_min_f(a.run_min, t);
            }
            const float d = qv - t, x = fabsf(d);
            const float sg = d > 0.f ? 1.f : (d < 0.f ? -1.f : 0.f);
            dq = a.inv_b * (x < 1.0f ? x : 1.0f) * sg;
            stg(a.td + 2 * b + h, x);
            if (a.q) stg(a.q + 2 * b + h, qv);
        }
        *p32(lds, a.F, r, 0) = dq;
    }
    __syncthreads();
    make_dp<P>(lds, a.F, 1, ACT_NONE, nullptr, 0, a.DP1, xt[6].part + (long)tile * 1, row0, B);
    __syncthreads();
    save_xt<P>(lds, a.DP1, 0, 1, xt[6].dp, a.ld, TR, row0);
    const GDesc nx1 = bwd_of(cr[4], 0);
    layer_bwd<P, TH>(lds, R, a.DP1, cr[6], 0, Hc, &nx1, a.act, y2, Hc, NO32, nullptr, 0, a.DP0,
                     xt[4].part + (long)tile * Hc, row0, B, si);
    save_xt<P>(lds, a.DP0, 0, Hc, xt[4].dp, a.ld, TR, row0);
    const GDesc nx2 = bwd_of(cr[2], 0);
    layer_bwd<P, TH>(lds, R, a.DP0, cr[4], 0, Hc, &nx2, a.act, y1, Hc, NO32, nullptr, 0, a.DP1,
                     xt[2].part + (long)tile * Hc, row0, B, si);
    save_xt<P>(lds, a.DP1, 0, Hc, xt[2].dp, a.ld, TR, row0);
    layer_bwd<P, TH>(lds, R, a.DP1, cr[2], 0, Hc, nullptr, ACT_NONE, nullptr, 0, a.DY, nullptr, 0, NO16, nullptr,
                     row0, B, si);
    norm_bwd<P>(lds, a.DY, a.H0, mean, Hc, 1e-8f, dot, a.DP0, xt[0].dp, a.ld, xt[0].part + (long)tile * Hc,
                row0, B);
}

struct EncoderArgs {
    Lin e[6];
    int act;
    const float *s, *a, *ns;
    int B, S, A, Z, He;
    float mse_scale;
    float *y0, *y1, *y2, *y3;
    XT xt[6];
    long ld;
    R16 X, H1, H2, CATZ, DP0, DP1;
    R32 H3, NZ, DY;
    int small_off;
    int lds_bytes;
    float *nz;
    int32_t *flag;
};

template <int P, int TH>
__global__ __launch_bounds__(NTH) void encoder_kernel(EncoderArgs a) {
    extern __shared__ __attribute__((aligned(16))) char lds[];
    const int row0 = blockIdx.x * TR, B = a.B, Z = a.Z, He = a.He, tile = blockIdx.x;
    const long ld = a.ld;
    const bool split = gridDim.y == 2, producer = split && blockIdx.y == 0;
    float *mean = (float *)(lds + a.small_off), *dot = mean + TR;
    int si = 0;
    FSTAMP(si);
    RowStage sns, sa, ss;
    if (!split || producer) row_issue(sns, a.ns, a.S, a.S, row0, B);
    if (!producer) {
        row_issue(sa, a.a, a.A, a.A, row0, B);
        row_issue(ss, a.s, a.S, a.S, row0, B);
    }
    u32x4 R[PD][TH];
    ring_fill(R, fwd_of(a.e[0]));
    zero_lds(lds, a.lds_bytes);
    __syncthreads();
    if (!split || producer) {
        row_put16<P>(lds, sns, a.X, 0, a.S, row0, B);
        if (!producer) row_put16<P>(lds, sa, a.CATZ, Z, a.A, row0, B);
        __syncthreads();
        layer_fwd<P, 1, TH>(lds, R, a.X, a.e[0], &a.e[1], a.act, a.H1, 0, NO32, nullptr, 0, row0, B, si);
        layer_fwd<P, 1, TH>(lds, R, a.H1, a.e[1], &a.e[2], a.act, a.H2, 0, NO32, nullptr, 0, row0, B, si);
        const GDesc z1 = fwd_of(a.e[0]);
        layer_fwd<P, 1, TH>(lds, R, a.H2, a.e[2], producer ? nullptr : &z1, ACT_NONE, NO16, 0, a.H3, nullptr, 0,
                            row0, B, si);
        norm_fwd<P>(lds, a.H3, Z, TR, 1e-8f, NO16, 0, NO16, 0, a.NZ, nullptr, 0, nullptr, nullptr, row0, B);
        __syncthreads();
        if (producer) {
            float *dst = a.nz + (long)row0 * Z;
            for (int k = threadIdx.x; k < TR * Z; k += NTH) {
                const int r = k / Z, c = k - r * Z;
                dst[k] = *p32(lds, a.NZ, r, c);
            }
            __threadfence();
            __syncthreads();
            if (threadIdx.x == 0) __hip_atomic_store(a.flag + tile, 1, __ATOMIC_RELEASE, __HIP_MEMORY_SCOPE_AGENT);
            return;
        }
    } else {
        row_put16<P>(lds, sa, a.CATZ, Z, a.A, row0, B);
    }
    row_put16<P>(lds, ss, a.X, 0, a.S, row0, B);
    __syncthreads();
    save_xt<P>(lds, a.X, 0, a.S, a.xt[0].x, ld, TR, row0);
    layer_fwd<P, 1, TH>(lds, R, a.X, a.e[0], &a.e[1], a.act, a.H1, 0, NO32, a.y0, He, row0, B, si);
    save_xt<P>(lds, a.H1, 0, He, a.xt[1].x, ld, TR, row0);
    layer_fwd<P, 1, TH>(lds, R, a.H1, a.e[1], &a.e[2], a.act, a.H2, 0, NO32, a.y1, He, row0, B, si);
    save_xt<P>(lds, a.H2, 0, He, a.xt[2].x, ld, TR, row0);
    layer_fwd<P, 1, TH>(lds, R, a.H2, a.e[2], &a.e[3], ACT_NONE, NO16, 0, a.H3, nullptr, 0, row0, B, si);
    norm_fwd<P>(lds, a.H3, Z, TR, 1e-8f, a.CATZ, 0, NO16, 0, NO32, nullptr, 0, mean, nullptr, row0, B);
    __syncthreads();
    save_xt<P>(lds, a.CATZ, 0, Z + a.A, a.xt[3].x, ld, TR, row0);
    layer_fwd<P, 1, TH>(lds, R, a.CATZ, a.e[3], &a.e[4], a.act, a.H1, 0, NO32, a.y2, He, row0, B, si);
    save_xt<P>(lds, a.H1, 0, He, a.xt[4].x, ld, TR, row0);
    const GDesc b6 = bwd_of(a.e[5], 0);
    layer_fwd<P, 1, TH>(lds, R, a.H1, a.e[4], &a.e[5], a.act, a.H2, 0, NO32, a.y3, He, row0, B, si);
    save_xt<P>(lds, a.H2, 0, He, a.xt[5].x, ld, TR, row0);
    layer_fwd<P, 1, TH>(lds, R, a.H2, a.e[5], &b6, ACT_NONE, NO16, 0, a.DY, nullptr, 0, row0, B, si);
    if (split) {
        if (threadIdx.x == 0) {
            while (__hip_atomic_load(a.flag + tile, __ATOMIC_ACQUIRE, __HIP_MEMORY_SCOPE_AGENT) == 0)
                __builtin_amdgcn_s_sleep(2);
            __hip_atomic_store(a.flag + tile, 0, __ATOMIC_RELAXED, __HIP_MEMORY_SCOPE_AGENT);
        }
        __syncthreads();
        __builtin_amdgcn_fence(__ATOMIC_ACQUIRE, "agent");
        const float *src = a.nz + (long)row0 * Z;
        for (int k = threadIdx.x; k < TR * Z; k += NTH) {
            const int r = k / Z, c = k - r * Z;
            *p32(lds, a.NZ, r, c) = src[k];
        }
        __syncthreads();
    }
    for (int k = threadIdx.x; k < TR * Z; k += NTH) {
        const int r = k / Z, c = k - r * Z;
        float *d = p32(lds, a.DY, r, c);
        *d = (*d - *p32(lds, a.NZ, r, c)) * a.mse_scale;
    }
    __syncthreads();
    make_dp<P>(lds, a.DY, Z, ACT_NONE, nullptr, 0, a.DP0, a.xt[5].part + (long)tile * Z, row0, B);
    __syncthreads();
    save_xt<P>(lds, a.DP0, 0, Z, a.xt[5].dp, ld, TR, row0);
    const GDesc nx3 = bwd_of(a.e[4], 0);
    layer_bwd<P, TH>(lds, R, a.DP0, a.e[5], 0, He, &nx3, a.act, a.y3, He, NO32, nullptr, 0, a.DP1,
                     a.xt[4].part + (long)tile * He, row0, B, si);
    save_xt<P>(lds, a.DP1, 0, He, a.xt[4].dp, ld, TR, row0);
    const GDesc nx4 = bwd_of(a.e[3], 0);
    layer_bwd<P, TH>(lds, R, a.DP1, a.e[4], 0, He, &nx4, a.act, a.y2, He, NO32, nullptr, 0, a.DP0,
                     a.xt[3].part + (long)tile * He, row0, B, si);
    save_xt<P>(lds, a.DP0, 0, He, a.xt[3].dp, ld, TR, row0);
    const GDesc nx5 = bwd_of(a.e[2], 0);
    layer_bwd<P, TH>(lds, R, a.DP0, a.e[3], 0, Z, &nx5, ACT_NONE, nullptr, 0, a.NZ, nullptr, 0, NO16, nullptr, row0, B,
                     si);
    norm_bwd<P>(lds, a.NZ, a.H3, mean, Z, 1e-8f, dot, a.DP1, a.xt[2].dp, ld, a.xt[2].part + (long)tile * Z, row0, B);
    __syncthreads();
    const GDesc nx6 = bwd_of(a.e[1], 0);
    layer_bwd<P, TH>(lds, R, a.DP1, a.e[2], 0, He, &nx6, a.act, a.y1, He, NO32, nullptr, 0, a.DP0,
                     a.xt[1].part + (long)tile * He, row0, B, si);
    save_xt<P>(lds, a.DP0, 0, He, a.xt[1].dp, ld, TR, row0);
    layer_bwd<P, TH>(lds, R, a.DP0, a.e[1], 0, He, nullptr, a.act, a.y0, He, NO32, nullptr, 0, a.DP1,
                     a.xt[0].part + (long)tile * He, row0, B, si);
    save_xt<P>(lds, a.DP1, 0, He, a.xt[0].dp, ld, TR, row0);
}

struct ActorArgs {
    Lin ac[4], fe[6], cr[8];
    int act_enc, act_actor, act_critic;
    const float *s, *zs;
    int B, S, A, Z, Ha, He, Hc;
    float dq;
    float *act_out;
    float *zsa_out;
    float *h0, *mean0;
    float *ya[2], *yz[2];
    float *yc[2];
    float *da, *dzsa;
    XT xt[4];
    long ld;
    R16 X, CATA, CATZ, CAT, H1, H2, DP0, DP1;
    R32 H0, DY, F, TW, TW2;
    int small_off;
    int lds;
};

template <int P, int TH>
__global__ __launch_bounds__(NTH) void actor_a_kernel(ActorArgs a) {
    extern __shared__ __attribute__((aligned(16))) char lds[];
    const int row0 = blockIdx.x * TR, B = a.B, Z = a.Z, Ha = a.Ha, He = a.He;
    const long ld = a.ld;
    int si = 0;
    RowStage ss, szs;
    ThinStage<THIN_NC> tw;
    row_issue(ss, a.s, a.S, a.S, row0, B);
    row_issue(szs, a.zs, Z, Z, row0, B);
    thin_issue(tw, a.ac[3].w, a.ac[3].ldw, 0, false, a.A, a.ac[3].K);
    u32x4 R[PD][TH];
    ring_fill(R, fwd_of(a.ac[0]));
    zero_lds(lds, a.lds);
    __syncthreads();
    row_put16<P>(lds, ss, a.X, 0, a.S, row0, B);
    row_put16<P>(lds, szs, a.CATA, Ha, Z, row0, B);
    row_put16<P>(lds, szs, a.CATZ, 0, Z, row0, B);
    thin_put<P>(lds, tw, a.TW, a.A, a.ac[3].K);
    __syncthreads();
    layer_fwd<P, 1, TH>(lds, R, a.X, a.ac[0], &a.ac[1], ACT_NONE, NO16, 0, a.H0, a.h0, Ha, row0, B, si);
    norm_fwd<P>(lds, a.H0, Ha, TR, 1e-8f, a.CATA, 0, NO16, 0, NO32, nullptr, 0, nullptr, a.mean0, row0, B);
    __syncthreads();
    save_xt<P>(lds, a.X, 0, a.S, a.xt[0].x, ld, TR, row0);
    save_xt<P>(lds, a.CATA, 0, Ha + Z, a.xt[1].x, ld, TR, row0);
    layer_fwd<P, 1, TH>(lds, R, a.CATA, a.ac[1], &a.ac[2], a.act_actor, a.H1, 0, NO32, a.ya[0], Ha, row0, B, si);
    layer_fwd<P, 1, TH>(lds, R, a.H1, a.ac[2], &a.fe[3], a.act_actor, a.H2, 0, NO32, a.ya[1], Ha, row0, B, si);
    save_xt<P>(lds, a.H1, 0, Ha, a.xt[2].x, ld, TR, row0);
    save_xt<P>(lds, a.H2, 0, Ha, a.xt[3].x, ld, TR, row0);
    layer_thin_fwd<P, THIN_NC>(lds, a.H2, a.ac[3], a.TW, ACT_TANH, a.F, TR, a.act_out, a.A, row0, B, si);
    for (int k = threadIdx.x; k < TR * a.A; k += NTH) {
        const int r = k / a.A, c = k - r * a.A;
        *pe<P>(lds, a.CATZ, r, Z + c) = Ty<P>::bits(*p32(lds, a.F, r, c));
    }
    __syncthreads();
    layer_fwd<P, 1, TH>(lds, R, a.CATZ, a.fe[3], &a.fe[4], a.act_enc, a.H1, 0, NO32, a.yz[0], He, row0, B, si);
    layer_fwd<P, 1, TH>(lds, R, a.H1, a.fe[4], &a.fe[5], a.act_enc, a.H2, 0, NO32, a.yz[1], He, row0, B, si);
    layer_fwd<P, 1, TH>(lds, R, a.H2, a.fe[5], (const Lin *)nullptr, ACT_NONE, NO16, 0, NO32, a.zsa_out, Z, row0, B, si);
}

template <int P, int TH>
__global__ __launch_bounds__(NTH) void actor_b_kernel(ActorArgs a) {
    extern __shared__ __attribute__((aligned(16))) char lds[];
    const int row0 = blockIdx.x * TR, B = a.B, Z = a.Z, h = blockIdx.y, Hc = a.Hc;
    const Lin *cr = a.cr + h;
    float *mean = (float *)(lds + a.small_off), *dot = mean + TR;
    float *y1 = a.yc[0] + (long)h * B * Hc, *y2 = a.yc[1] + (long)h * B * Hc;
    int si = 0;
    FSTAMP(si);
    RowStage ss, sa, sz, szs;
    ThinStage<THIN_NC> tw;
    row_issue(ss, a.s, a.S, a.S, row0, B);
    row_issue(sa, a.act_out, a.A, a.A, row0, B);
    row_issue(sz, a.zsa_out, Z, Z, row0, B);
    row_issue(szs, a.zs, Z, Z, row0, B);
    thin_issue(tw, cr[0].w, cr[0].ldw, a.S, true, a.A, Hc);
    u32x4 R[PD][TH];
    ring_fill(R, fwd_of(cr[0]));
    zero_lds(lds, a.lds);
    __syncthreads();
    row_put16<P>(lds, ss, a.X, 0, a.S, row0, B);
    row_put16<P>(lds, sa, a.X, a.S, a.A, row0, B);
    row_put16<P>(lds, sz, a.CAT, Hc, Z, row0, B);
    row_put16<P>(lds, szs, a.CAT, Hc + Z, Z, row0, B);
    if constexpr (P != PREC_F32) thin_put<P>(lds, tw, a.TW, a.A, Hc);
    __syncthreads();
    layer_fwd<P, 1, TH>(lds, R, a.X, cr[0], &cr[2], ACT_NONE, NO16, 0, a.H0, nullptr, 0, row0, B, si);
    norm_fwd<P>(lds, a.H0, Hc, TR, 1e-8f, a.CAT, 0, NO16, 0, NO32, nullptr, 0, mean, nullptr, row0, B);
    __syncthreads();
    layer_fwd<P, 1, TH>(lds, R, a.CAT, cr[2], &cr[4], a.act_critic, a.H1, 0, NO32, y1, Hc, row0, B, si);
    if constexpr (P == PREC_F32) thin_put<P>(lds, tw, a.TW, a.A, Hc);
    const GDesc b3 = bwd_of(cr[6], 0);
    layer_fwd<P, 1, TH>(lds, R, a.H1, cr[4], &b3, a.act_critic, a.H2, 0, NO32, y2, Hc, row0, B, si);
    for (int r = threadIdx.x; r < TR; r += NTH) *p32(lds, a.F, r, 0) = a.dq;
    __syncthreads();
    make_dp<P>(lds, a.F, 1, ACT_NONE, nullptr, 0, a.DP1, nullptr, row0, B);
    __syncthreads();
    const GDesc nx7 = bwd_of(cr[4], 0);
    layer_bwd<P, TH>(lds, R, a.DP1, cr[6], 0, Hc, &nx7, a.act_critic, y2, Hc, NO32, nullptr, 0, a.DP0, nullptr, row0,
                     B, si);
    const GDesc nx8 = bwd_of(cr[2], Hc);
    layer_bwd<P, TH>(lds, R, a.DP0, cr[4], 0, Hc, &nx8, a.act_critic, y1, Hc, NO32, nullptr, 0, a.DP1, nullptr, row0,
                     B, si);
    const GDesc nx9 = bwd_of(cr[2], 0);
    layer_bwd<P, TH>(lds, R, a.DP1, cr[2], Hc, Hc + Z, &nx9, ACT_NONE, nullptr, 0, NO32,
                     a.dzsa + (long)h * B * Z, Z, NO16, nullptr, row0, B, si);
    layer_bwd<P, TH>(lds, R, a.DP1, cr[2], 0, Hc, nullptr, ACT_NONE, nullptr, 0, a.DY, nullptr, 0, NO16, nullptr,
                     row0, B, si);
    FSTAMP(si);
    norm_bwd<P>(lds, a.DY, a.H0, mean, Hc, 1e-8f, dot, a.DP0, nullptr, 0, nullptr, row0, B);
    __syncthreads();
    FSTAMP(si);
    thin<P, THIN_NC>(lds, a.DP0, 0, Hc, a.TW, a.A, a.F, 1.f / Ty<P>::gs);
    __syncthreads();
    FSTAMP(si);
    for (int k = threadIdx.x; k < TR * a.A; k += NTH) {
        const int r = k / a.A, c = k - r * a.A;
        if (row0 + r < B) stg(a.da + ((long)h * B + row0 + r) * a.A + c, *p32(lds, a.F, r, c));
    }
}

template <int P, int TH>
__global__ __launch_bounds__(NTH) void actor_c_kernel(ActorArgs a) {
    extern __shared__ __attribute__((aligned(16))) char lds[];
    const int row0 = blockIdx.x * TR, B = a.B, Z = a.Z, Ha = a.Ha, He = a.He, A = a.A, tile = blockIdx.x;
    const long ld = a.ld;
    float *mean = (float *)(lds + a.small_off), *dot = mean + TR;
    int si = 0;
    FSTAMP(si);
    RowStage d0, d1, sh;
    ThinStage<THIN_NC> tw;
    row_issue(d0, a.dzsa, Z, Z, row0, B);
    row_issue(d1, a.dzsa + (long)B * Z, Z, Z, row0, B);
    row_issue(sh, a.h0, Ha, Ha, row0, B);
    const float m0 = ldg(a.mean0 + min(row0 + (int)(threadIdx.x % TR), B - 1));
    thin_issue(tw, a.fe[3].w, a.fe[3].ldw, Z, true, A, He);
    u32x4 R[PD][TH];
    ring_fill(R, bwd_of(a.fe[5], 0));
    zero_lds(lds, a.lds);
    __syncthreads();
    row_add(d0, d1);
    row_put16<P>(lds, d0, a.DP0, 0, Z, row0, B, Ty<P>::gs);
    if (threadIdx.x < TR) mean[threadIdx.x] = row0 + (int)threadIdx.x < B ? m0 : 0.f;
    row_put32(lds, sh, a.H0, Ha, row0, B);
    thin_put<P>(lds, tw, a.TW, A, He);
    __syncthreads();
    const GDesc nx10 = bwd_of(a.fe[4], 0);
    layer_bwd<P, TH>(lds, R, a.DP0, a.fe[5], 0, He, &nx10, a.act_enc, a.yz[1], He, NO32, nullptr, 0, a.DP1, nullptr,
                     row0, B, si);
    const GDesc nx11 = bwd_of(a.ac[3], 0);
    layer_bwd<P, TH>(lds, R, a.DP1, a.fe[4], 0, He, &nx11, a.act_enc, a.yz[0], He, NO32, nullptr, 0, a.DP0, nullptr,
                     row0, B, si);
    FSTAMP(si);
    thin<P, THIN_NC>(lds, a.DP0, 0, He, a.TW, A, a.F, 1.f / Ty<P>::gs);
    __syncthreads();
    FSTAMP(si);
    for (int k = threadIdx.x; k < TR * A; k += NTH) {
        const int r = k / A, c = k - r * A, b = row0 + r;
        float v = 0.f;
        if (b < B) {
            const float y = ldg(a.act_out + (long)b * A + c);
            v = (*p32(lds, a.F, r, c) + ldg(a.da + (long)b * A + c) + ldg(a.da + ((long)B + b) * A + c)) * (1.f - y * y);
        }
        *p32(lds, a.F, r, c) = v;
    }
    __syncthreads();
    make_dp<P>(lds, a.F, A, ACT_NONE, nullptr, 0, a.DP1, a.xt[3].part + (long)tile * A, row0, B);
    __syncthreads();
    save_xt<P>(lds, a.DP1, 0, A, a.xt[3].dp, ld, TR, row0);
    const GDesc nx12 = bwd_of(a.ac[2], 0);
    layer_bwd<P, TH>(lds, R, a.DP1, a.ac[3], 0, Ha, &nx12, a.act_actor, a.ya[1], Ha, NO32, nullptr, 0, a.DP0,
                     a.xt[2].part + (long)tile * Ha, row0, B, si);
    save_xt<P>(lds, a.DP0, 0, Ha, a.xt[2].dp, ld, TR, row0);
    const GDesc nx13 = bwd_of(a.ac[1], 0);
    layer_bwd<P, TH>(lds, R, a.DP0, a.ac[2], 0, Ha, &nx13, a.act_actor, a.ya[0], Ha, NO32, nullptr, 0, a.DP1,
                     a.xt[1].part + (long)tile * Ha, row0, B, si);
    save_xt<P>(lds, a.DP1, 0, Ha, a.xt[1].dp, ld, TR, row0);
    layer_bwd<P, TH>(lds, R, a.DP1, a.ac[1], 0, Ha, nullptr, ACT_NONE, nullptr, 0, a.DY, nullptr, 0, NO16, nullptr,
                     row0, B, si);
    FSTAMP(si);
    norm_bwd<P>(lds, a.DY, a.H0, mean, Ha, 1e-8f, dot, a.DP0, a.xt[0].dp, ld, a.xt[0].part + (long)tile * Ha, row0,
                B);
    __syncthreads();
    FSTAMP(si);
}

struct WgJob {
    const char *dp, *x;
    const float *part;
    float *dw, *db;
    int N, K, tiles_k, ntiles_rows;
    int first;
    long w_off, b_off;
    u32x4 *wf, *wb;
    int ksf, ksb, opt;
    int vec;
};
struct WgOpt {
    float *p, *m, *v, *step;
    float lr, b1, b2, eps, wd;
};
struct WgArgs {
    int njobs, total;
    long ld;
    int rows;
    const float *td;
    float *prio;
    int B;
    float alpha, minp;
    WgJob j[TD7F_MAX_WG];
    WgOpt o[TD7_ADAM_MAX_OPT];
    int nopt;
    uint32_t *ticket;
    int xcd;
};

constexpr int PD2 = 8;

template <int P, bool ADAM>
__global__ __launch_bounds__(256, 2) void wgrad_kernel(WgArgs a) {
    if ((int)blockIdx.x == a.total) {
        for (int b = threadIdx.x; b < a.B; b += 256)
            stg(a.prio + b, powf(fmaxf(fmaxf(ldg(a.td + 2 * b), ldg(a.td + 2 * b + 1)), a.minp), a.alpha));
    } else {
    const int b = a.xcd ? xcd_contiguous((int)blockIdx.x, a.total) : (int)blockIdx.x;
    int q = 0;
    while (q + 1 < a.njobs && b >= a.j[q + 1].first) ++q;
    const WgJob &J = a.j[q];
    const int t = b - J.first;
    const int n0 = (t / J.tiles_k) * 64, k0 = (t % J.tiles_k) * 64;
    const int w = threadIdx.x >> 6, lane = threadIdx.x & 63;
    const int wn = n0 + 32 * (w >> 1), wk = k0 + 32 * (w & 1);
    const int vr = threadIdx.x >> 4, vc = 4 * (threadIdx.x & 15);
    const long ld = a.ld;
    constexpr int KD = Ty<P>::KD;
    const char *ap[2], *bp2[2];
#pragma unroll
    for (int u = 0; u < 2; ++u) {
        ap[u] = J.dp + ((long)((wn + 16 * u) >> 4) * (ld / KD)) * 1024 + lane * 16;
        bp2[u] = J.x + ((long)((wk + 16 * u) >> 4) * (ld / KD)) * 1024 + lane * 16;
    }
    floatx4 acc[2][2];
#pragma unroll
    for (int u = 0; u < 2; ++u)
#pragma unroll
        for (int v = 0; v < 2; ++v) acc[u][v] = floatx4{0.f, 0.f, 0.f, 0.f};
    const int ns = a.rows / KD;
    u32x4 fa[PD2][2], fb[PD2][2];
#pragma unroll
    for (int p = 0; p < PD2; ++p)
#pragma unroll
        for (int u = 0; u < 2; ++u) {
            fa[p][u] = ldg((const u32x4 *)(ap[u] + 1024 * p));
            fb[p][u] = ldg((const u32x4 *)(bp2[u] + 1024 * p));
            __builtin_amdgcn_sched_barrier(0);
        }
    float ss = 0.f, bc = 1.f;
    float pp[16], mm[16], vv[16], bp = 0.f, bm = 0.f, bv = 0.f;
    if constexpr (ADAM) {
        const WgOpt &o = a.o[J.opt];
        if (J.vec) {
#pragma unroll
            for (int h = 0; h < 4; ++h) {
                const int n = n0 + vr + 16 * h, k = k0 + vc;
                floatx4 p4{0.f, 0.f, 0.f, 0.f}, m4 = p4, v4 = p4;
                if (n < J.N && k < J.K) {
                    const long i = J.w_off + (long)n * J.K + k;
                    p4 = ldg((const floatx4 *)(o.p + i)), m4 = ldg((const floatx4 *)(o.m + i));
                    v4 = ldg((const floatx4 *)(o.v + i));
                }
#pragma unroll
                for (int j = 0; j < 4; ++j) pp[4 * h + j] = p4[j], mm[4 * h + j] = m4[j], vv[4 * h + j] = v4[j];
            }
        } else {
#pragma unroll
            for (int u = 0; u < 2; ++u)
#pragma unroll
                for (int v = 0; v < 2; ++v)
#pragma unroll
                    for (int e = 0; e < 4; ++e) {
                        const int n = wn + 16 * u + 4 * (lane >> 4) + e, k = wk + 16 * v + (lane & 15);
                        const long i = J.w_off + ((n < J.N && k < J.K) ? (long)n * J.K + k : 0);
                        const int x = (2 * u + v) * 4 + e;
                        pp[x] = ldg(o.p + i), mm[x] = ldg(o.m + i), vv[x] = ldg(o.v + i);
                    }
        }
        if (k0 == 0 && J.db && w == 0) {
            const long i = J.b_off + (n0 + lane < J.N ? n0 + lane : 0);
            bp = ldg(o.p + i), bm = ldg(o.m + i), bv = ldg(o.v + i);
        }
        __builtin_amdgcn_sched_barrier(0);
        const float st = *o.step + 1.0f;
        ss = o.lr / (1.0f - powf(o.b1, st));
        bc = sqrtf(1.0f - powf(o.b2, st));
    }
    int s0 = 0;
    for (; s0 + PD2 < ns; s0 += PD2) {
#pragma unroll
        for (int p = 0; p < PD2; ++p) {
            const int s = s0 + p;
#pragma unroll
            for (int j = 0; j < Ty<P>::SUB; ++j)
#pragma unroll
                for (int u = 0; u < 2; ++u)
#pragma unroll
                    for (int v = 0; v < 2; ++v) acc[u][v] = Ty<P>::mfma(fa[p][u], fb[p][v], acc[u][v], j);
            __builtin_amdgcn_sched_barrier(0);
#pragma unroll
            for (int u = 0; u < 2; ++u) {
                fa[p][u] = ldg((const u32x4 *)(ap[u] + 1024L * (s + PD2)));
                fb[p][u] = ldg((const u32x4 *)(bp2[u] + 1024L * (s + PD2)));
                __builtin_amdgcn_sched_barrier(0);
            }
        }
    }
#pragma unroll
    for (int p = 0; p < PD2; ++p)
#pragma unroll
        for (int j = 0; j < Ty<P>::SUB; ++j)
#pragma unroll
            for (int u = 0; u < 2; ++u)
#pragma unroll
                for (int v = 0; v < 2; ++v) acc[u][v] = Ty<P>::mfma(fa[p][u], fb[p][v], acc[u][v], j);
    __shared__ alignas(16) typename Ty<P>::E T[ADAM ? 64 : 1][Ty<P>::EB == 4 ? 68 : 72];
    __shared__ alignas(16) float G[64][68];
    if (J.vec) {
#pragma unroll
        for (int u = 0; u < 2; ++u)
#pragma unroll
            for (int v = 0; v < 2; ++v)
#pragma unroll
                for (int e = 0; e < 4; ++e)
                    G[wn - n0 + 16 * u + 4 * (lane >> 4) + e][wk - k0 + 16 * v + (lane & 15)] =
                        acc[u][v][e] * (1.f / Ty<P>::gs);
        __syncthreads();
#pragma unroll
        for (int h = 0; h < 4; ++h) {
            const int r = vr + 16 * h, n = n0 + r, k = k0 + vc;
            const bool ok = n < J.N && k < J.K;
            const floatx4 g4 = *(const floatx4 *)&G[r][vc];
            if (ok) stg((floatx4 *)(J.dw + (long)n * J.K + k), g4);
            if constexpr (ADAM) {
                const WgOpt &o = a.o[J.opt];
                float pw[4];
#pragma unroll
                for (int j = 0; j < 4; ++j) {
                    const int x = 4 * h + j;
                    adam_one(pp[x], g4[j], mm[x], vv[x], ss, bc, o.b1, o.b2, o.eps, o.wd, 1.0f);
                    pw[j] = ok ? pp[x] : 0.f;
                }
                if (ok) {
                    const long i = J.w_off + (long)n * J.K + k;
                    stg((floatx4 *)(o.p + i), floatx4{pp[4 * h], pp[4 * h + 1], pp[4 * h + 2], pp[4 * h + 3]});
                    stg((floatx4 *)(o.m + i), floatx4{mm[4 * h], mm[4 * h + 1], mm[4 * h + 2], mm[4 * h + 3]});
                    stg((floatx4 *)(o.v + i), floatx4{vv[4 * h], vv[4 * h + 1], vv[4 * h + 2], vv[4 * h + 3]});
                }
                if constexpr (Ty<P>::EB == 4) *(floatx4 *)&T[r][vc] = floatx4{pw[0], pw[1], pw[2], pw[3]};
                else *(u32x2 *)&T[r][vc] = pack4<P>(pw);
            }
        }
    } else {
#pragma unroll
    for (int u = 0; u < 2; ++u)
#pragma unroll
        for (int v = 0; v < 2; ++v) {
            const int k = wk + 16 * v + (lane & 15);
#pragma unroll
            for (int e = 0; e < 4; ++e) {
                const int n = wn + 16 * u + 4 * (lane >> 4) + e;
                const bool ok = n < J.N && k < J.K;
                const float g = acc[u][v][e] * (1.f / Ty<P>::gs);
                if (ok) stg(J.dw + (long)n * J.K + k, g);
                if constexpr (ADAM) {
                    const WgOpt &o = a.o[J.opt];
                    const int x = (2 * u + v) * 4 + e;
                    adam_one(pp[x], g, mm[x], vv[x], ss, bc, o.b1, o.b2, o.eps, o.wd, 1.0f);
                    if (ok) {
                        const long i = J.w_off + (long)n * J.K + k;
                        stg(o.p + i, pp[x]), stg(o.m + i, mm[x]), stg(o.v + i, vv[x]);
                    }
                    T[n - n0][k - k0] = Ty<P>::bits(ok ? pp[x] : 0.f);
                }
            }
        }
    }
    if (k0 == 0 && J.db) {
        __shared__ float red[4][64];
        const int n = n0 + lane;
        float sacc = 0.f;
        if (n < J.N) {
#pragma unroll 8
            for (int r = w; r < J.ntiles_rows; r += 4) sacc += ldg(J.part + (long)r * J.N + n);
        }
        red[w][lane] = sacc;
        __syncthreads();
        if (w == 0 && n < J.N) {
            const float g = ((red[0][lane] + red[1][lane]) + red[2][lane]) + red[3][lane];
            stg(J.db + n, g);
            if constexpr (ADAM) {
                const WgOpt &o = a.o[J.opt];
                adam_one(bp, g, bm, bv, ss, bc, o.b1, o.b2, o.eps, o.wd, 1.0f);
                stg(o.p + J.b_off + n, bp), stg(o.m + J.b_off + n, bm), stg(o.v + J.b_off + n, bv);
            }
        }
    }
    if constexpr (ADAM && P == PREC_F32) {
        __syncthreads();
#pragma unroll
        for (int h = 0; h < 4; ++h) {
            const int i = threadIdx.x + 256 * h;
            const int r = i >> 4, c = 4 * (i & 15);
            const int n = n0 + r, k = k0 + c;
            if (n < J.N && k < J.K)
                stg(J.wf + ((long)(n >> 4) * J.ksf + (k >> 4)) * 64 + (n & 15) + 16 * ((k & 15) >> 2),
                    *(const u32x4 *)&T[r][c]);
        }
        if (J.wb) {
#pragma unroll
            for (int h = 0; h < 4; ++h) {
                const int i = threadIdx.x + 256 * h;
                const int c = i & 63, r4 = 4 * (i >> 6);
                const int n = n0 + r4, k = k0 + c;
                if (n < J.N && k < J.K)
                    stg(J.wb + ((long)(k >> 4) * J.ksb + (n >> 4)) * 64 + (k & 15) + 16 * ((n & 15) >> 2),
                        __builtin_bit_cast(u32x4, floatx4{T[r4][c], T[r4 + 1][c], T[r4 + 2][c], T[r4 + 3][c]}));
            }
        }
    } else if constexpr (ADAM) {
        __syncthreads();
#pragma unroll
        for (int h = 0; h < 2; ++h) {
            const int i = threadIdx.x + 256 * h;
            const int r = i >> 3, c = 8 * (i & 7);
            const int n = n0 + r, k = k0 + c;
            if (n < J.N && k < J.K)
                stg(J.wf + ((long)(n >> 4) * J.ksf + (k >> 5)) * 64 + (n & 15) + 16 * ((k & 31) >> 3),
                    *(const u32x4 *)&T[r][c]);
        }
        if (J.wb) {
#pragma unroll
            for (int h = 0; h < 2; ++h) {
                const int i = threadIdx.x + 256 * h;
                const int c = i & 63, r8 = 8 * (i >> 6);
                const int n = n0 + r8, k = k0 + c;
                if (n < J.N && k < J.K) {
                    uint32_t d[4];
#pragma unroll
                    for (int jj = 0; jj < 4; ++jj) d[jj] = (uint32_t)T[r8 + 2 * jj][c] | ((uint32_t)T[r8 + 2 * jj + 1][c] << 16);
                    stg(J.wb + ((long)(k >> 4) * J.ksb + (n >> 5)) * 64 + (k & 15) + 16 * ((n & 31) >> 3),
                        u32x4{d[0], d[1], d[2], d[3]});
                }
            }
        }
    }
    }
    if constexpr (ADAM) {
        __syncthreads();
        if (threadIdx.x == 0) {
            const uint32_t done = atomicAdd(a.ticket, 1u);
            if (done == gridDim.x - 1) {
                for (int k = 0; k < a.nopt; ++k) *a.o[k].step = *a.o[k].step + 1.0f;
                *a.ticket = 0u;
            }
        }
    }
}

}

using namespace td7f;

static XT xt_of(const td7f_xt &x) { return XT{x.x, x.dp, x.part}; }

static bool env_on(const char *name) {
    const char *e = getenv(name);
    return !(e && e[0] == '0' && e[1] == 0);
}
static bool al16(const void *p) { return ((uintptr_t)p & 15) == 0; }
static bool prec_ok(int p) { return p == PREC_BF16 || p == PREC_F16 || p == PREC_F32; }
static bool xt_ok(const td7f_xt *xt, int n) {
    for (int i = 0; i < n; ++i)
        if (!xt[i].x || !xt[i].dp || !xt[i].part) return false;
    return true;
}
static bool alias_pair(R16 r, int ld, R16 &d0, R16 &d1) {
    d0 = R16{r.off, ld};
    d1 = R16{r.off + round_up(TR * ld * 2, 16), ld};
    return d1.off + TR * ld * 2 <= r.off + TR * r.ld * 2;
}
static bool alias32(R16 a, R16 b, int n, R32 &d) {
    d = R32{a.off, n};
    return a.off + TR * n * 4 <= b.off + TR * b.ld * 2;
}
static bool wb_ok(const td7f_lin *l, int n) {
    for (int i = 0; i < n; ++i)
        if (!l[i].wb || l[i].ksb <= 0 || l[i].ksb % PD) return false;
    return true;
}

extern "C" {

#ifdef EXO_STAMPS
int td7f_train_debug_set_stamps(unsigned long long *buf) {
    return hipMemcpyToSymbol(HIP_SYMBOL(g_td7f_stamps), &buf, sizeof(buf)) == hipSuccess ? 0 : -5;
}
#endif

int td7f_critic(int32_t prec, const int32_t *act, const td7f_lin *critic, const float *s, const float *a,
                const float *zs, const float *zsa, const float *qt, const float *reward, const float *not_done,
                float discount, const float *lo, const float *hi, float *run_max, float *run_min, int32_t B,
                int32_t S, int32_t A, float *td, float *q, float *y1, float *y2, const td7f_xt *xt, int64_t ld,
                void *stream) {
    return td7f_critic_phase(0, prec, act, critic, s, a, zs, zsa, qt, reward, not_done, discount, lo, hi, run_max,
                             run_min, B, S, A, td, q, y1, y2, xt, ld, nullptr, nullptr, nullptr, stream);
}

int td7f_critic_phase(int32_t phase, int32_t prec, const int32_t *act, const td7f_lin *critic, const float *s,
                      const float *a, const float *zs, const float *zsa, const float *qt, const float *reward,
                      const float *not_done, float discount, const float *lo, const float *hi, float *run_max,
                      float *run_min, int32_t B, int32_t S, int32_t A, float *td, float *q, float *y1, float *y2,
                      const td7f_xt *xt, int64_t ld, float *q_ws, float *h0_ws, float *mean_ws, void *stream) {
    if (!prec_ok(prec) || !act || !critic || !s || !a || !zs || !zsa || !qt || !reward || !not_done || !lo || !hi ||
        !run_max || !run_min || !td || !y1 || !y2 || !xt || B <= 0 || S <= 0 || S > NTH || A <= 0 || A > THIN_NC || ld < B || ld % 32)
        return EXO_EINVAL;
    if (phase < 0 || phase > 2 || (phase != 0 && (!q_ws || !h0_ws || !mean_ws))) return EXO_EINVAL;
    const int th = th_of(critic, 8);
    if ((th != 4 && th != 5) || !wb_ok(critic, 8) || !xt_ok(xt, 8)) return EXO_EINVAL;
    CriticArgs g{};
    for (int i = 0; i < 8; ++i) {
        g.cr[i] = lin_of(critic[i]);
        g.xt[i] = xt_of(xt[i]);
    }
    g.act = act[2];
    g.s = s; g.a = a; g.zs = zs; g.zsa = zsa; g.qt = qt; g.reward = reward; g.not_done = not_done;
    g.discount = discount;
    g.inv_b = 1.0f / (float)B;
    g.lo = lo; g.hi = hi; g.run_max = run_max; g.run_min = run_min;
    g.B = B; g.S = S; g.A = A;
    g.Hc = critic[0].n_out;
    g.Z = (critic[2].n_in - g.Hc) / 2;
    if (critic[0].n_in != S + A || critic[4].n_in != g.Hc || critic[6].n_in != g.Hc || critic[6].n_out != 1 ||
        g.Z * 2 + g.Hc != critic[2].n_in || g.Hc % 16 || g.Hc > 320)
        return EXO_EINVAL;
    g.td = td; g.q = q; g.y1 = y1; g.y2 = y2; g.ld = ld;
    g.phase = phase;
    g.qs = q_ws; g.h0s = h0_ws; g.ms = mean_ws;
    const int kd = kd_of(prec);
    Bump b(1);
    g.X = b.r16(TR, ld16(S + A, kd));
    g.CAT = b.r16(TR, ld16(g.Hc + 2 * g.Z, kd));
    g.H1 = b.r16(TR, ld16(g.Hc, kd));
    g.H2 = b.r16(TR, ld16(g.Hc, kd));
    if (prec == PREC_F32) {
        if (!alias_pair(g.CAT, ld16(g.Hc, kd), g.DP0, g.DP1) || !alias32(g.H1, g.H2, g.Hc, g.DY)) return EXO_EINVAL;
    } else {
        g.DP0 = b.r16(TR, ld16(g.Hc));
        g.DP1 = b.r16(TR, ld16(g.Hc));
    }
    g.H0 = b.r32(TR, g.Hc);
    if (prec != PREC_F32) g.DY = b.r32(TR, g.Hc);
    g.F = b.r32(TR, 16);
    g.TW = b.r32(1, g.Hc);
    const R32 sm = b.r32(1, 2 * TR);
    g.small_off = sm.off;
    g.lds_bytes = b.off;
    return DISPATCH(prec, th, critic_kernel, dim3((B + TR - 1) / TR, 2), b.off, g, (hipStream_t)stream);
}

int td7f_encoder(int32_t prec, const int32_t *act, const td7f_lin *enc, const float *s, const float *a,
                 const float *ns, int32_t B, float *const *y, const td7f_xt *xt, int64_t ld, float *nz_ws,
                 int32_t *flag_ws, void *stream) {
    if (!prec_ok(prec) || !act || !enc || !s || !a || !ns || !y || !xt || B <= 0 || ld < B || ld % 32 ||
        (!nz_ws) != (!flag_ws))
        return EXO_EINVAL;
    const int th = th_of(enc, 6);
    if ((th != 4 && th != 5) || !wb_ok(enc, 6) || !xt_ok(xt, 6)) return EXO_EINVAL;
    EncoderArgs g{};
    for (int i = 0; i < 6; ++i) {
        g.e[i] = lin_of(enc[i]);
        g.xt[i] = xt_of(xt[i]);
    }
    if (!y[0] || !y[1] || !y[2] || !y[3]) return EXO_EINVAL;
    g.y0 = y[0];
    g.y1 = y[1];
    g.y2 = y[2];
    g.y3 = y[3];
    g.act = act[0];
    g.s = s; g.a = a; g.ns = ns;
    g.B = B;
    g.S = enc[0].n_in;
    g.He = enc[0].n_out;
    g.Z = enc[2].n_out;
    g.A = enc[3].n_in - g.Z;
    if (g.A <= 0 || g.A > THIN_NC || g.S > NTH || enc[1].n_out != g.He || enc[4].n_out != g.He || enc[5].n_out != g.Z || g.Z % 4)
        return EXO_EINVAL;
    g.mse_scale = 2.0f / ((float)B * (float)g.Z);
    g.ld = ld;
    const int w = std::max(g.Z, g.He), kd = kd_of(prec);
    Bump b(1);
    g.X = b.r16(TR, ld16(g.S, kd));
    g.H1 = b.r16(TR, ld16(g.He, kd));
    g.H2 = b.r16(TR, ld16(g.He, kd));
    g.CATZ = b.r16(TR, ld16(g.Z + g.A, kd));
    if (prec == PREC_F32 && ld16(w, kd) <= g.H1.ld) {
        g.DP0 = R16{g.H1.off, ld16(w, kd)};
        g.DP1 = R16{g.H2.off, ld16(w, kd)};
    } else {
        g.DP0 = b.r16(TR, ld16(w, kd));
        g.DP1 = b.r16(TR, ld16(w, kd));
    }
    g.H3 = b.r32(TR, g.Z);
    g.NZ = b.r32(TR, w);
    g.DY = b.r32(TR, w);
    const R32 sm = b.r32(1, 2 * TR);
    g.small_off = sm.off;
    g.lds_bytes = b.off;
    g.nz = nz_ws;
    g.flag = flag_ws;
    return DISPATCH(prec, th, encoder_kernel, dim3((B + TR - 1) / TR, nz_ws ? 2 : 1), b.off, g, (hipStream_t)stream);
}

int td7f_actor(int32_t prec, int32_t phase, const int32_t *act, const td7f_lin *actor, const td7f_lin *fenc,
               const td7f_lin *critic, const float *s, const float *zs, int32_t B, const td7f_actor_bufs *bufs,
               const td7f_xt *xt, int64_t ld, void *stream) {
    if (!prec_ok(prec) || phase < 0 || phase > 2 || !act || !actor || !fenc || !critic || !s || !zs || !bufs || !xt ||
        B <= 0 || ld < B || ld % 32)
        return EXO_EINVAL;
    td7f_lin all[18];
    for (int i = 0; i < 4; ++i) all[i] = actor[i];
    for (int i = 0; i < 6; ++i) all[4 + i] = fenc[i];
    for (int i = 0; i < 8; ++i) all[10 + i] = critic[i];
    const int th = th_of(all, 18);
    if ((th != 4 && th != 5) || !xt_ok(xt, 4)) return EXO_EINVAL;
    if (phase == 1 && !wb_ok(critic, 8)) return EXO_EINVAL;
    if (phase == 2 && (!wb_ok(actor, 4) || !wb_ok(fenc + 3, 3))) return EXO_EINVAL;
    const td7f_actor_bufs &u = *bufs;
    if (!u.act_out || !u.zsa_out || !u.h0 || !u.mean0 || !u.ya[0] || !u.ya[1] || !u.yz[0] || !u.yz[1] ||
        !u.yc[0] || !u.yc[1] || !u.da || !u.dzsa)
        return EXO_EINVAL;
    ActorArgs g{};
    for (int i = 0; i < 4; ++i) {
        g.ac[i] = lin_of(actor[i]);
        g.xt[i] = xt_of(xt[i]);
    }
    for (int i = 0; i < 6; ++i) g.fe[i] = lin_of(fenc[i]);
    for (int i = 0; i < 8; ++i) g.cr[i] = lin_of(critic[i]);
    g.act_enc = act[0]; g.act_actor = act[1]; g.act_critic = act[2];
    g.s = s; g.zs = zs; g.B = B;
    g.S = actor[0].n_in;
    g.A = actor[3].n_out;
    g.Ha = actor[0].n_out;
    g.Z = fenc[2].n_out;
    g.He = fenc[3].n_out;
    g.Hc = critic[0].n_out;
    if (actor[1].n_in != g.Ha + g.Z || fenc[3].n_in != g.Z + g.A || critic[0].n_in != g.S + g.A ||
        critic[2].n_in != g.Hc + 2 * g.Z || g.A > THIN_NC || g.S > NTH || g.Hc % 16 || g.Ha % 16)
        return EXO_EINVAL;
    g.dq = -1.0f / (2.0f * (float)B);
    g.act_out = u.act_out; g.zsa_out = u.zsa_out; g.h0 = u.h0; g.mean0 = u.mean0;
    for (int i = 0; i < 2; ++i) {
        g.ya[i] = u.ya[i];
        g.yz[i] = u.yz[i];
        g.yc[i] = u.yc[i];
    }
    g.da = u.da; g.dzsa = u.dzsa; g.ld = ld;
    const int hmax = std::max(g.Ha, std::max(g.He, g.Hc)), kd = kd_of(prec);
    Bump b(1);
    if (phase == 0) {
        g.X = b.r16(TR, ld16(g.S, kd));
        g.CATA = b.r16(TR, ld16(g.Ha + g.Z, kd));
        g.CATZ = b.r16(TR, ld16(g.Z + g.A, kd));
        g.H1 = b.r16(TR, ld16(hmax, kd));
        g.H2 = b.r16(TR, ld16(hmax, kd));
        g.H0 = b.r32(TR, g.Ha);
        g.F = b.r32(TR, 16);
        g.TW = b.r32(THIN_NC, g.Ha);
    } else if (phase == 1) {
        g.X = b.r16(TR, ld16(g.S + g.A, kd));
        g.CAT = b.r16(TR, ld16(g.Hc + 2 * g.Z, kd));
        g.H1 = b.r16(TR, ld16(g.Hc, kd));
        g.H2 = b.r16(TR, ld16(g.Hc, kd));
        if (prec == PREC_F32) {
            if (!alias_pair(g.CAT, ld16(g.Hc, kd), g.DP0, g.DP1) || !alias32(g.H1, g.H2, g.Hc, g.DY)) return EXO_EINVAL;
            const int tw = g.DP1.off + round_up(TR * g.DP1.ld * 2, 16);
            g.TW = R32{tw, g.Hc};
            if (tw + THIN_NC * g.Hc * 4 > g.CAT.off + TR * g.CAT.ld * 2) return EXO_EINVAL;
        } else {
            g.DP0 = b.r16(TR, ld16(g.Hc));
            g.DP1 = b.r16(TR, ld16(g.Hc));
        }
        g.H0 = b.r32(TR, g.Hc);
        if (prec != PREC_F32) g.DY = b.r32(TR, g.Hc);
        g.F = b.r32(TR, 16);
        if (prec != PREC_F32) g.TW = b.r32(THIN_NC, g.Hc);
    } else {
        g.DP0 = b.r16(TR, ld16(std::max(hmax, g.Z), kd));
        g.DP1 = b.r16(TR, ld16(std::max(hmax, g.Z), kd));
        g.H0 = b.r32(TR, g.Ha);
        g.DY = b.r32(TR, g.Ha);
        g.F = b.r32(TR, 16);
        g.TW = b.r32(THIN_NC, g.He);
    }
    const R32 sm = b.r32(1, 2 * TR);
    g.small_off = sm.off;
    g.lds = b.off;
    const hipStream_t st = (hipStream_t)stream;
    const dim3 grid((B + TR - 1) / TR, phase == 1 ? 2 : 1);
    if (phase == 0) return DISPATCH(prec, th, actor_a_kernel, grid, b.off, g, st);
    if (phase == 1) return DISPATCH(prec, th, actor_b_kernel, grid, b.off, g, st);
    return DISPATCH(prec, th, actor_c_kernel, grid, b.off, g, st);
}

static int wgrad_args(int32_t prec, int32_t njobs, const td7f_wg_job *jobs, int64_t ld, int32_t rows,
                      const float *td, float *prio, int32_t B, float alpha, float min_priority, WgArgs &g) {
    if (!prec_ok(prec) || njobs <= 0 || njobs > TD7F_MAX_WG || !jobs || rows <= 0 || rows % (32 * PD2) ||
        ld < rows || ld % 32 || (prio && (!td || B <= 0)))
        return EXO_EINVAL;
    g.njobs = njobs;
    g.ld = ld;
    g.rows = rows;
    const bool vec = env_on("EXO_WGRAD_VEC");
    int total = 0;
    for (int q = 0; q < njobs; ++q) {
        const td7f_wg_job &J = jobs[q];
        if (!J.dp || !J.x || !J.dw || J.n <= 0 || J.k <= 0 || (J.db && (!J.part || J.row_tiles <= 0))) return EXO_EINVAL;
        WgJob &w = g.j[q];
        w.dp = (const char *)J.dp;
        w.x = (const char *)J.x;
        w.part = J.part;
        w.dw = J.dw;
        w.db = J.db;
        w.N = J.n;
        w.K = J.k;
        w.tiles_k = (J.k + 63) / 64;
        w.ntiles_rows = J.row_tiles;
        w.first = total;
        w.vec = vec && J.k % 4 == 0 && al16(J.dw);
        total += ((J.n + 63) / 64) * w.tiles_k;
    }
    g.total = total;
    g.xcd = env_on("EXO_WGRAD_XCD");
    g.td = td;
    g.prio = prio;
    g.B = B;
    g.alpha = alpha;
    g.minp = min_priority;
    return EXO_OK;
}

int td7f_wgrad(int32_t prec, int32_t njobs, const td7f_wg_job *jobs, int64_t ld, int32_t rows, const float *td,
               float *prio, int32_t B, float alpha, float min_priority, void *stream) {
    WgArgs g{};
    const int rc = wgrad_args(prec, njobs, jobs, ld, rows, td, prio, B, alpha, min_priority, g);
    if (rc != EXO_OK) return rc;
    const hipStream_t st = (hipStream_t)stream;
    const dim3 grid(g.total + (prio ? 1 : 0));
    if (prec == PREC_BF16) hipLaunchKernelGGL((wgrad_kernel<PREC_BF16, false>), grid, dim3(256), 0, st, g);
    else if (prec == PREC_F16) hipLaunchKernelGGL((wgrad_kernel<PREC_F16, false>), grid, dim3(256), 0, st, g);
    else hipLaunchKernelGGL((wgrad_kernel<PREC_F32, false>), grid, dim3(256), 0, st, g);
    return hipGetLastError() == hipSuccess ? EXO_OK : EXO_EDEVICE;
}

int td7f_wgrad_adam(int32_t prec, int32_t njobs, const td7f_wg_job *jobs, int64_t ld, int32_t rows, const float *td,
                    float *prio, int32_t B, float alpha, float min_priority, int32_t nopt, float *const *p,
                    float *const *m, float *const *v, float *const *step, const float *lr, const float *beta1,
                    const float *beta2, const float *eps, const float *weight_decay, const td7f_wg_adam *adam,
                    uint32_t *ticket, void *stream) {
    WgArgs g{};
    const int rc = wgrad_args(prec, njobs, jobs, ld, rows, td, prio, B, alpha, min_priority, g);
    if (rc != EXO_OK) return rc;
    if (nopt <= 0 || nopt > TD7_ADAM_MAX_OPT || !adam || !ticket) return EXO_EINVAL;
    g.nopt = nopt;
    g.ticket = ticket;
    for (int k = 0; k < nopt; ++k) {
        if (!p[k] || !m[k] || !v[k] || !step[k]) return EXO_EINVAL;
        g.o[k] = WgOpt{p[k], m[k], v[k], step[k], lr[k], beta1[k], beta2[k], eps[k], weight_decay[k]};
    }
    for (int q = 0; q < njobs; ++q) {
        const td7f_wg_adam &A = adam[q];
        const td7f_wg_job &J = jobs[q];
        if (A.opt < 0 || A.opt >= nopt || A.w_off < 0 || A.b_off < 0 || !J.db || !A.wf ||
            A.ksf * kd_of(prec) < J.k || (A.wb && A.ksb * kd_of(prec) < J.n))
            return EXO_EINVAL;
        WgJob &w = g.j[q];
        w.w_off = A.w_off;
        w.b_off = A.b_off;
        const WgOpt &o = g.o[A.opt];
        w.vec = w.vec && A.w_off % 4 == 0 && al16(o.p) && al16(o.m) && al16(o.v);
        w.wf = (u32x4 *)A.wf;
        w.wb = (u32x4 *)A.wb;
        w.ksf = A.ksf;
        w.ksb = A.wb ? A.ksb : 0;
        w.opt = A.opt;
    }
    const hipStream_t st = (hipStream_t)stream;
    const dim3 grid(g.total + (prio ? 1 : 0));
    if (prec == PREC_BF16) hipLaunchKernelGGL((wgrad_kernel<PREC_BF16, true>), grid, dim3(256), 0, st, g);
    else if (prec == PREC_F16) hipLaunchKernelGGL((wgrad_kernel<PREC_F16, true>), grid, dim3(256), 0, st, g);
    else hipLaunchKernelGGL((wgrad_kernel<PREC_F32, true>), grid, dim3(256), 0, st, g);
    return hipGetLastError() == hipSuccess ? EXO_OK : EXO_EDEVICE;
}

}
```

Baseline: 17.36 million.

## Split GEMM by output tiles across wave groups instead of K-split reduction

Rewrites the fused MLP GEMM so each wave group owns half of the output tiles and walks the full K range, instead of splitting K across two wave groups and summing the partials through LDS. The weight ring now holds half the tiles but twice the prefetch depth. This removes the LDS reduction buffer from every layer's LDS layout, and the barrier after the GEMM is kept only when the epilogue output overlaps the input buffer. In exchange, each wave issues a longer serial MFMA chain per output tile. The original K-split rounding is kept by taking an accumulator snapshot at the split point.

```diff
diff --git a/a-deep-reinforcement-learning-enabled-soft-exoskeleton-for-parkinson-s-patients_amd/csrc/td7_fused.h b/a-deep-reinforcement-learning-enabled-soft-exoskeleton-for-parkinson-s-patients_amd/csrc/td7_fused.h
--- a/a-deep-reinforcement-learning-enabled-soft-exoskeleton-for-parkinson-s-patients_amd/csrc/td7_fused.h
+++ b/a-deep-reinforcement-learning-enabled-soft-exoskeleton-for-parkinson-s-patients_amd/csrc/td7_fused.h
@@ -94,23 +94,30 @@
     int t0;
 };
 
-__device__ __forceinline__ void kgroup_range(int ks, int kg, int &kb, int &ke) {
-    const int kA = ks >= 2 * PD ? ((ks / 2 + PD - 1) / PD) * PD : ks;
-    kb = kg ? kA : 0;
-    ke = kg ? ks : kA;
-}
-
+constexpr int RD = 2 * PD;
+constexpr int os_of(int th) { return (th + 1) / 2; }
 template <int TH>
-__device__ __forceinline__ void ring_fill(u32x4 (&R)[PD][TH], const GDesc &g) {
-    const int wv = threadIdx.x >> 6, w = wv % NW, kg = wv / NW, lane = threadIdx.x & 63;
-    int kb, ke;
-    kgroup_range(g.ks, kg, kb, ke);
-    const bool live = ke > kb;
-#pragma unroll
-    for (int p = 0; p < PD; ++p)
-#pragma unroll
-        for (int i = 0; i < TH; ++i) {
-            R[p][i] = ldg(g.wp + (live ? ((size_t)(g.t0 + w + NW * i) * g.ks + kb + p) * 64 : 0) + lane);
+using Ring = u32x4[RD][os_of(TH)];
+
+__device__ __forceinline__ int wave_id() { return __builtin_amdgcn_readfirstlane((int)(threadIdx.x >> 6)); }
+template <int TH>
+__device__ __forceinline__ int own_slot(int j) {
+    return j + (wave_id() / NW) * os_of(TH);
+}
+
+__device__ __forceinline__ int kchain_split(int ks) { return ks >= 2 * PD ? ((ks / 2 + PD - 1) / PD) * PD : ks; }
+
+template <int TH>
+__device__ __forceinline__ void ring_fill(Ring<TH> &R, const GDesc &g) {
+    constexpr int OS = os_of(TH);
+    const int w = wave_id() % NW, lane = threadIdx.x & 63;
+#pragma unroll
+    for (int p = 0; p < RD; ++p)
+#pragma unroll
+        for (int j = 0; j < OS; ++j) {
+            const int i = own_slot<TH>(j);
+            R[p][j] = u32x4{0u, 0u, 0u, 0u};
+            if (i < TH && (p < PD || g.ks >= RD)) R[p][j] = ldg(g.wp + ((size_t)(g.t0 + w + NW * i) * g.ks + p) * 64 + lane);
             __builtin_amdgcn_sched_barrier(0);
         }
 }
@@ -121,123 +128,116 @@
     int c0, row0, nrows, ncols;
 };
 template <int RT, int TH>
-__device__ __forceinline__ void epi_prefetch(const EpiSrc &e, int t0, floatx4 (&ep)[RT][TH]) {
-#pragma unroll
-    for (int i = 0; i < TH; ++i) {
-        const int wv = threadIdx.x >> 6;
-        const int col = 16 * (t0 + wv % NW + NW * i) + 4 * ((threadIdx.x & 63) >> 4) - e.c0;
-        const bool mine = (i < (TH + 1) / 2) == (wv < NW);
+__device__ __forceinline__ void epi_prefetch(const EpiSrc &e, int t0, floatx4 (&ep)[RT][os_of(TH)]) {
+#pragma unroll
+    for (int j = 0; j < os_of(TH); ++j) {
+        const int i = own_slot<TH>(j);
+        const int col = 16 * (t0 + wave_id() % NW + NW * i) + 4 * ((threadIdx.x & 63) >> 4) - e.c0;
 #pragma unroll
         for (int r = 0; r < RT; ++r) {
             const int row = (threadIdx.x & 15) + TR * r;
-            const bool ok = e.p && mine && col >= 0 && col < e.ncols && (e.ld == 0 || e.row0 + row < e.nrows);
-            ep[r][i] = ok ? ldg((const floatx4 *)(e.p + (e.ld ? (long)(e.row0 + row) * e.ld : 0) + col))
+            const bool ok = e.p && i < TH && col >= 0 && col < e.ncols && (e.ld == 0 || e.row0 + row < e.nrows);
+            ep[r][j] = ok ? ldg((const floatx4 *)(e.p + (e.ld ? (long)(e.row0 + row) * e.ld : 0) + col))
                           : floatx4{0.f, 0.f, 0.f, 0.f};
         }
     }
 }
 
 template <int P, int RT, int TH>
-__device__ __forceinline__ void gemm(char *lds, int a_off, int lda, const GDesc &g, u32x4 (&R)[PD][TH],
-                                     floatx4 (&acc)[RT][TH], const GDesc *next, const EpiSrc &es,
-                                     floatx4 (&ep)[RT][TH]) {
-    const int wv = threadIdx.x >> 6, w = wv % NW, kg = wv / NW, lane = threadIdx.x & 63;
-    int kb, ke, nb = 0, ne = 0;
-    kgroup_range(g.ks, kg, kb, ke);
-    if (next) kgroup_range(next->ks, kg, nb, ne);
-    epi_prefetch(es, g.t0, ep);
+__device__ __forceinline__ void kstep(Ring<TH> &R, int p, const char *ap, int lda, int s, int n, u32x4 (&an)[RT],
+                                      floatx4 (&acc)[RT][os_of(TH)]) {
+    u32x4 x[RT];
+    const int sn = s + 1 < n ? s + 1 : n - 1;
+#pragma unroll
+    for (int r = 0; r < RT; ++r) {
+        x[r] = an[r];
+        an[r] = *(const u32x4 *)(ap + (r * TR * lda + 32 * sn) * 2);
+    }
+#pragma unroll
+    for (int j = 0; j < Ty<P>::SUB; ++j)
+#pragma unroll
+        for (int i = 0; i < os_of(TH); ++i) {
+#pragma unroll
+            for (int r = 0; r < RT; ++r) acc[r][i] = Ty<P>::mfma(R[p][i], x[r], acc[r][i], j);
+            __builtin_amdgcn_sched_barrier(0);
+        }
+}
+
+template <int P, int RT, int TH>
+__device__ __forceinline__ void gemm(char *lds, int a_off, int lda, const GDesc &g, Ring<TH> &R,
+                                     floatx4 (&acc)[RT][os_of(TH)], const GDesc *next, const EpiSrc &es,
+                                     floatx4 (&ep)[RT][os_of(TH)], bool sync) {
+    constexpr int OS = os_of(TH);
+    const int w = wave_id() % NW, lane = threadIdx.x & 63;
+    const int n = g.ks, kA = kchain_split(n), nk = next ? next->ks : 0;
+    epi_prefetch<RT, TH>(es, g.t0, ep);
+    floatx4 first[RT][OS];
 #pragma unroll
     for (int r = 0; r < RT; ++r)
 #pragma unroll
-        for (int i = 0; i < TH; ++i) acc[r][i] = floatx4{0.f, 0.f, 0.f, 0.f};
-    if (ke > kb) {
-        const u32x4 *bp[TH];
-#pragma unroll
-        for (int i = 0; i < TH; ++i) bp[i] = g.wp + ((size_t)(g.t0 + w + NW * i) * g.ks + kb) * 64 + lane;
-        const char *ap = lds + a_off + ((lane & 15) * lda + 8 * (lane >> 4) + 32 * kb) * 2;
-        const int n = ke - kb;
-        u32x4 an[RT];
-#pragma unroll
-        for (int r = 0; r < RT; ++r) an[r] = *(const u32x4 *)(ap + r * TR * lda * 2);
-        int s0 = 0;
-        for (; s0 + PD < n; s0 += PD) {
-#pragma unroll
-            for (int p = 0; p < PD; ++p) {
-                const int s = s0 + p;
-                u32x4 x[RT];
-#pragma unroll
-                for (int r = 0; r < RT; ++r) {
-                    x[r] = an[r];
-                    an[r] = *(const u32x4 *)(ap + (r * TR * lda + 32 * (s + 1)) * 2);
-                }
-#pragma unroll
-                for (int j = 0; j < Ty<P>::SUB; ++j)
-#pragma unroll
-                    for (int i = 0; i < TH; ++i) {
-#pragma unroll
-                        for (int r = 0; r < RT; ++r) acc[r][i] = Ty<P>::mfma(R[p][i], x[r], acc[r][i], j);
-                        __builtin_amdgcn_sched_barrier(0);
-                    }
-#pragma unroll
-                for (int i = 0; i < TH; ++i) {
-                    R[p][i] = ldg(bp[i] + (s + PD) * 64);
+        for (int j = 0; j < OS; ++j) acc[r][j] = first[r][j] = floatx4{0.f, 0.f, 0.f, 0.f};
+    bool own[OS];
+    const u32x4 *bp[OS], *np[OS];
+#pragma unroll
+    for (int j = 0; j < OS; ++j) {
+        const int i = own_slot<TH>(j);
+        own[j] = i < TH;
+        const int t = w + NW * (own[j] ? i : 0);
+        bp[j] = g.wp + (size_t)(g.t0 + t) * n * 64 + lane;
+        np[j] = next ? next->wp + (size_t)(next->t0 + t) * nk * 64 + lane : bp[j];
+    }
+    const char *ap = lds + a_off + ((lane & 15) * lda + 8 * (lane >> 4)) * 2;
+    u32x4 an[RT];
+#pragma unroll
+    for (int r = 0; r < RT; ++r) an[r] = *(const u32x4 *)(ap + r * TR * lda * 2);
+    int s0 = 0;
+    for (; n - s0 > RD; s0 += RD) {
+        const bool more = n - s0 >= 2 * RD;
+#pragma unroll
+        for (int p = 0; p < RD; ++p) {
+            if (p % PD == 0 && s0 + p == kA) {
+#pragma unroll
+                for (int r = 0; r < RT; ++r)
+#pragma unroll
+                    for (int j = 0; j < OS; ++j) first[r][j] = acc[r][j], acc[r][j] = floatx4{0.f, 0.f, 0.f, 0.f};
+            }
+            kstep<P, RT, TH>(R, p, ap, lda, s0 + p, n, an, acc);
+            if (p < PD || more) {
+#pragma unroll
+                for (int j = 0; j < OS; ++j) {
+                    if (own[j]) R[p][j] = ldg(bp[j] + (size_t)(s0 + p + RD) * 64);
                     __builtin_amdgcn_sched_barrier(0);
                 }
             }
         }
-        const u32x4 *np[TH];
-        if (ne > nb)
-#pragma unroll
-            for (int i = 0; i < TH; ++i) np[i] = next->wp + ((size_t)(next->t0 + w + NW * i) * next->ks + nb) * 64 + lane;
-#pragma unroll
-        for (int p = 0; p < PD; ++p) {
-            const int s = s0 + p;
-            u32x4 x[RT];
-#pragma unroll
-            for (int r = 0; r < RT; ++r) {
-                x[r] = an[r];
-                if (p + 1 < PD) an[r] = *(const u32x4 *)(ap + (r * TR * lda + 32 * (s + 1)) * 2);
-            }
-#pragma unroll
-            for (int j = 0; j < Ty<P>::SUB; ++j)
-#pragma unroll
-                for (int i = 0; i < TH; ++i) {
-#pragma unroll
-                    for (int r = 0; r < RT; ++r) acc[r][i] = Ty<P>::mfma(R[p][i], x[r], acc[r][i], j);
-                    __builtin_amdgcn_sched_barrier(0);
-                }
-            if (ne > nb) {
-#pragma unroll
-                for (int i = 0; i < TH; ++i) {
-                    R[p][i] = ldg(np[i] + p * 64);
-                    __builtin_amdgcn_sched_barrier(0);
-                }
-            }
-        }
-    } else if (next) {
-        ring_fill(R, *next);
-    }
-    constexpr int h = (TH + 1) / 2;
-    floatx4 *red = (floatx4 *)lds + ((w * 64 + lane) * RT) * TH;
+    }
+    const bool full = n - s0 == RD;
+#pragma unroll
+    for (int p = 0; p < RD; ++p) {
+        if (p < PD || full) {
+            if (p % PD == 0 && s0 + p == kA && kA < n) {
+#pragma unroll
+                for (int r = 0; r < RT; ++r)
+#pragma unroll
+                    for (int j = 0; j < OS; ++j) first[r][j] = acc[r][j], acc[r][j] = floatx4{0.f, 0.f, 0.f, 0.f};
+            }
+            kstep<P, RT, TH>(R, p, ap, lda, s0 + p, n, an, acc);
+        }
+        if (next && (p < PD || nk >= RD)) {
+#pragma unroll
+            for (int j = 0; j < OS; ++j) {
+                if (own[j]) R[p][j] = ldg(np[j] + p * 64);
+                __builtin_amdgcn_sched_barrier(0);
+            }
+        }
+    }
+    if (sync) __syncthreads();
 #pragma unroll
     for (int r = 0; r < RT; ++r)
 #pragma unroll
-        for (int i = 0; i < TH; ++i)
-            if ((i < h) != (kg == 0)) red[r * TH + i] = acc[r][i];
-    __syncthreads();
-#pragma unroll
-    for (int r = 0; r < RT; ++r)
-#pragma unroll
-        for (int i = 0; i < TH; ++i)
-            if ((i < h) == (kg == 0)) acc[r][i] += red[r * TH + i];
-}
-
-constexpr int red_bytes(int rt, int tpw) { return NW * 64 * rt * tpw * 16; }
-
-template <int TH>
-__device__ __forceinline__ bool owns(int i) {
-    return (i < (TH + 1) / 2) == ((threadIdx.x >> 6) < NW);
-}
+        for (int j = 0; j < OS; ++j) acc[r][j] += first[r][j];
+}
+
 __device__ __forceinline__ int acc_col(int t0, int i) {
     const int wv = threadIdx.x >> 6;
     return 16 * (t0 + wv % NW + NW * i) + 4 * ((threadIdx.x & 63) >> 4);
@@ -274,13 +274,14 @@
 }
 
 template <int P, int RT, int TH>
-__device__ __forceinline__ void epi_fwd(char *lds, const floatx4 (&acc)[RT][TH], const floatx4 (&bias)[RT][TH], int N,
-                                        int act, R16 o16, int col0, R32 o32, float *g, long gld, int row0,
-                                        int nrows) {
-#pragma unroll
-    for (int i = 0; i < TH; ++i) {
-        if (!owns<TH>(i)) continue;
-        const int n = acc_col(0, i);
+__device__ __forceinline__ void epi_fwd(char *lds, const floatx4 (&acc)[RT][os_of(TH)],
+                                        const floatx4 (&bias)[RT][os_of(TH)], int N, int act, R16 o16, int col0,
+                                        R32 o32, float *g, long gld, int row0, int nrows) {
+#pragma unroll
+    for (int i = 0; i < os_of(TH); ++i) {
+        const int slot = own_slot<TH>(i);
+        if (slot >= TH) continue;
+        const int n = acc_col(0, slot);
         if (n >= N) continue;
         const floatx4 b = bias[0][i];
 #pragma unroll
@@ -297,13 +298,14 @@
 }
 
 template <int P, int RT, int TH>
-__device__ __forceinline__ void epi_bwd(char *lds, const floatx4 (&acc)[RT][TH], int t0, int c0, int c1, int act,
-                                        const floatx4 (&yv_)[RT][TH], R32 o32, float *g, long gld, R16 o16,
-                                        float *part, int row0, int nrows) {
-#pragma unroll
-    for (int i = 0; i < TH; ++i) {
-        if (!owns<TH>(i)) continue;
-        const int col = acc_col(t0, i);
+__device__ __forceinline__ void epi_bwd(char *lds, const floatx4 (&acc)[RT][os_of(TH)], int t0, int c0, int c1,
+                                        int act, const floatx4 (&yv_)[RT][os_of(TH)], R32 o32, float *g, long gld,
+                                        R16 o16, float *part, int row0, int nrows) {
+#pragma unroll
+    for (int i = 0; i < os_of(TH); ++i) {
+        const int slot = own_slot<TH>(i);
+        if (slot >= TH) continue;
+        const int col = acc_col(t0, slot);
         const bool in = col >= c0 && col < c1;
         const int m = col - c0;
         float cs[4] = {0.f, 0.f, 0.f, 0.f};
@@ -404,7 +406,7 @@
 __device__ __forceinline__ void row_issue(RowStage &s, const float *src, long sld, int ncols, int row0, int nrows) {
     const int c = min((int)threadIdx.x, ncols - 1);
 #pragma unroll
-    for (int r = 0; r < TR; ++r) s.v[r] = ldg(src + (long)(row0 + r < nrows ? row0 + r : row0) * sld + c);
+    for (int r = 0; r < TR; ++r) s.v[r] = ldg(src + (long)min(row0 + r, nrows - 1) * sld + c);
 }
 __device__ __forceinline__ void row_add(RowStage &s, const RowStage &o) {
 #pragma unroll
@@ -626,20 +628,28 @@
 #endif
 
 
+__device__ __forceinline__ bool epi_aliases(R16 a, int rows, R16 o16, R32 o32) {
+    const int a0 = a.off, a1 = a.off + rows * a.ld * 2;
+    const bool h16 = o16.off >= 0 && o16.off < a1 && a0 < o16.off + rows * o16.ld * 2;
+    const bool h32 = o32.off >= 0 && o32.off < a1 && a0 < o32.off + rows * o32.ld * 4;
+    return h16 || h32;
+}
+
 template <int P, int RT, int TH>
-__device__ __forceinline__ void layer_fwd(char *lds, u32x4 (&R)[PD][TH], R16 a, const Lin &L, const GDesc *next,
+__device__ __forceinline__ void layer_fwd(char *lds, Ring<TH> &R, R16 a, const Lin &L, const GDesc *next,
                                           int act, R16 o16, int col0, R32 o32, float *g, long gld, int row0,
                                           int nrows, int &si) {
     FSTAMP(si);
-    floatx4 acc[RT][TH], bias[RT][TH];
+    floatx4 acc[RT][os_of(TH)], bias[RT][os_of(TH)];
     const GDesc gd{L.wf, L.ksf, 0};
-    gemm<P, RT, TH>(lds, a.off, a.ld, gd, R, acc, next, EpiSrc{L.b, 0, 0, 0, 0, L.N}, bias);
+    gemm<P, RT, TH>(lds, a.off, a.ld, gd, R, acc, next, EpiSrc{L.b, 0, 0, 0, 0, L.N}, bias,
+                    epi_aliases(a, RT * TR, o16, o32));
     FSTAMP(si);
     epi_fwd<P, RT, TH>(lds, acc, bias, L.N, act, o16, col0, o32, g, gld, row0, nrows);
     __syncthreads();
 }
 template <int P, int RT, int TH>
-__device__ __forceinline__ void layer_fwd(char *lds, u32x4 (&R)[PD][TH], R16 a, const Lin &L, const Lin *next, int act,
+__device__ __forceinline__ void layer_fwd(char *lds, Ring<TH> &R, R16 a, const Lin &L, const Lin *next, int act,
                                           R16 o16, int col0, R32 o32, float *g, long gld, int row0, int nrows,
                                           int &si) {
     GDesc gn{nullptr, 0, 0};
@@ -713,8 +723,7 @@
 inline int ld16(int n, int kd = 32) { return ks_of(n, kd) * 32 + 16; }
 
 struct Bump {
-    int off;
-    explicit Bump(int rt) : off(red_bytes(rt, 5)) {}
+    int off = 0;
     R16 r16(int rows, int ld) {
         R16 r{off, ld};
         off += round_up(rows * ld * 2, 16);
diff --git a/a-deep-reinforcement-learning-enabled-soft-exoskeleton-for-parkinson-s-patients_amd/csrc/td7_fused.hip b/a-deep-reinforcement-learning-enabled-soft-exoskeleton-for-parkinson-s-patients_amd/csrc/td7_fused.hip
--- a/a-deep-reinforcement-learning-enabled-soft-exoskeleton-for-parkinson-s-patients_amd/csrc/td7_fused.hip
+++ b/a-deep-reinforcement-learning-enabled-soft-exoskeleton-for-parkinson-s-patients_amd/csrc/td7_fused.hip
@@ -277,8 +277,8 @@
 };
 
 #define RING_START(first)      \
-    u32x4 R[PD][TH];           \
-    ring_fill(R, GDesc{(first).wf, (first).ksf, 0})
+    Ring<TH> R;                \
+    ring_fill<TH>(R, GDesc{(first).wf, (first).ksf, 0})
 
 __device__ __forceinline__ R16 rows_of(R16 r, int t) { return R16{r.off + t * TR * r.ld * 2, r.ld}; }
 __device__ __forceinline__ R32 rows_of(R32 r, int t) { return R32{r.off + t * TR * r.ld * 4, r.ld}; }
@@ -344,7 +344,10 @@
     layer_fwd<P, RT, TH>(lds, R, a.X, a.ac[0], &a.ac[1], ACT_NONE, NO16, 0, a.F, nullptr, 0, row0, a.n, si);
     norm_fwd<P>(lds, a.F, a.Ha, rows, 1e-8f, a.CAT, 0, NO16, 0, NO32, nullptr, 0, nullptr, nullptr, row0, a.n);
     __syncthreads();
-    if (a.F.off == a.H1.off) zero_lds(lds + a.H1.off, a.H2.off + rows * a.H2.ld * 2 - a.H1.off);
+    if (a.F.off == a.H1.off) {
+        zero_lds(lds + a.H1.off, a.H2.off + rows * a.H2.ld * 2 - a.H1.off);
+        __syncthreads();
+    }
     layer_fwd<P, RT, TH>(lds, R, a.CAT, a.ac[1], &a.ac[2], a.act_actor, a.H1, 0, NO32, nullptr, 0, row0, a.n, si);
     layer_fwd<P, RT, TH>(lds, R, a.H1, a.ac[2], (const Lin *)nullptr, a.act_actor, a.H2, 0, NO32, nullptr, 0, row0, a.n, si);
     if constexpr (RT == 1) {
@@ -673,7 +676,7 @@
                    : rt_env && (rt_env[0] == '1' || rt_env[0] == '2') ? rt_env[0] - '0'
                    : rt ? rt : (n > 8192 ? 2 : 1);
     const int rows = RT * TR, hmax = std::max(enc[0].n_out, std::max(enc[1].n_out, std::max(a.Ha, actor[1].n_out)));
-    Bump b(RT);
+    Bump b;
     a.X = b.r16(rows, ld16(a.S, kd));
     a.H1 = b.r16(rows, ld16(hmax, kd));
     a.H2 = b.r16(rows, ld16(hmax, kd));
@@ -759,7 +762,7 @@
     const int old = eh * round_up(2 * a.Z + a.A, 8);
     const int fld = std::max(hmax, 16);
     const bool wide_out = prec == PREC_F32 && old > ld16(a.Ha + a.Z, kd);
-    Bump ba(1);
+    Bump ba;
     a.X = ba.r16(rows, ld16(a.S + a.A, kd));
     if (wide_out) a.CATA = ba.r16(rows, ld16(a.Ha + a.Z, kd));
     a.H1 = ba.r16(rows, ld16(hmax, kd));
@@ -777,7 +780,7 @@
     }
     a.TW = ba.r32(THIN_NC, tactor[3].n_in);
     a.lds_a = ba.off;
-    Bump bb(1);
+    Bump bb;
     const R16 Xb = bb.r16(rows, ld16(a.S + a.A, kd)), H1b = bb.r16(rows, ld16(hmax, kd)), H2b = bb.r16(rows, ld16(hmax, kd));
     const R16 CATb = bb.r16(rows, ld16(a.Hc + 2 * a.Z, kd));
     const R32 Fb = bb.r32(rows, std::max(hmax, 16));
@@ -817,7 +820,7 @@
     const int rows = TR;
     int hmax = 0;
     for (int i = 0; i < 6; ++i) hmax = std::max(hmax, fenc[i].n_out);
-    Bump b(1);
+    Bump b;
     a.X = b.r16(rows, ld16(a.S, kd));
     a.H1 = b.r16(rows, ld16(hmax, kd));
     a.H2 = b.r16(rows, ld16(hmax, kd));
diff --git a/a-deep-reinforcement-learning-enabled-soft-exoskeleton-for-parkinson-s-patients_amd/csrc/td7_fused_train.hip b/a-deep-reinforcement-learning-enabled-soft-exoskeleton-for-parkinson-s-patients_amd/csrc/td7_fused_train.hip
--- a/a-deep-reinforcement-learning-enabled-soft-exoskeleton-for-parkinson-s-patients_amd/csrc/td7_fused_train.hip
+++ b/a-deep-reinforcement-learning-enabled-soft-exoskeleton-for-parkinson-s-patients_amd/csrc/td7_fused_train.hip
@@ -13,14 +13,15 @@
 };
 
 template <int P, int TH>
-__device__ __forceinline__ void layer_bwd(char *lds, u32x4 (&R)[PD][TH], R16 a, const Lin &L, int c0, int c1,
+__device__ __forceinline__ void layer_bwd(char *lds, Ring<TH> &R, R16 a, const Lin &L, int c0, int c1,
                                           const GDesc *next, int act, const float *y, long yld, R32 o32, float *g,
                                           long gld, R16 o16, float *part, int row0, int nrows, int &si) {
     FSTAMP(si);
-    floatx4 acc[1][TH], yv[1][TH];
+    floatx4 acc[1][os_of(TH)], yv[1][os_of(TH)];
     const GDesc gd{L.wb, L.ksb, c0 / 16};
     gemm<P, 1, TH>(lds, a.off, a.ld, gd, R, acc, next,
-                   EpiSrc{act != ACT_NONE ? y : nullptr, yld, c0, row0, nrows, c1 - c0}, yv);
+                   EpiSrc{act != ACT_NONE ? y : nullptr, yld, c0, row0, nrows, c1 - c0}, yv,
+                   epi_aliases(a, TR, o16, o32));
     FSTAMP(si);
     epi_bwd<P, 1, TH>(lds, acc, c0 / 16, c0, c1, act, yv, o32, g, gld, o16, part, row0, nrows);
     __syncthreads();
@@ -68,7 +69,7 @@
     float *y1 = a.y1 + (long)h * B * Hc, *y2 = a.y2 + (long)h * B * Hc;
     int si = 0;
     FSTAMP(si);
-    u32x4 R[PD][TH];
+    Ring<TH> R;
     const long Bp = (long)gridDim.x * TR;
     if (a.phase == 2) {
         constexpr int PER = TR * 320 / NTH;
@@ -81,7 +82,7 @@
         }
         const float qv = threadIdx.x < TR ? ldg(a.qs + h * Bp + row0 + threadIdx.x) : 0.f;
         const float mv = threadIdx.x < TR ? ldg(a.ms + h * Bp + row0 + threadIdx.x) : 0.f;
-        ring_fill(R, bwd_of(cr[6], 0));
+        ring_fill<TH>(R, bwd_of(cr[6], 0));
         zero_lds(lds, a.lds_bytes);
         __syncthreads();
 #pragma unroll
@@ -102,7 +103,7 @@
     row_issue(sz, a.zsa, Z, Z, row0, B);
     row_issue(szs, a.zs, Z, Z, row0, B);
     thin_issue(tw, cr[6].w, cr[6].ldw, 0, false, 1, cr[6].K);
-    ring_fill(R, fwd_of(cr[0]));
+    ring_fill<TH>(R, fwd_of(cr[0]));
     zero_lds(lds, a.lds_bytes);
     __syncthreads();
     row_put16<P>(lds, ss, a.X, 0, a.S, row0, B);
@@ -203,8 +204,8 @@
         row_issue(sa, a.a, a.A, a.A, row0, B);
         row_issue(ss, a.s, a.S, a.S, row0, B);
     }
-    u32x4 R[PD][TH];
-    ring_fill(R, fwd_of(a.e[0]));
+    Ring<TH> R;
+    ring_fill<TH>(R, fwd_of(a.e[0]));
     zero_lds(lds, a.lds_bytes);
     __syncthreads();
     if (!split || producer) {
@@ -326,8 +327,8 @@
     row_issue(ss, a.s, a.S, a.S, row0, B);
     row_issue(szs, a.zs, Z, Z, row0, B);
     thin_issue(tw, a.ac[3].w, a.ac[3].ldw, 0, false, a.A, a.ac[3].K);
-    u32x4 R[PD][TH];
-    ring_fill(R, fwd_of(a.ac[0]));
+    Ring<TH> R;
+    ring_fill<TH>(R, fwd_of(a.ac[0]));
     zero_lds(lds, a.lds);
     __syncthreads();
     row_put16<P>(lds, ss, a.X, 0, a.S, row0, B);
@@ -371,8 +372,8 @@
     row_issue(sz, a.zsa_out, Z, Z, row0, B);
     row_issue(szs, a.zs, Z, Z, row0, B);
     thin_issue(tw, cr[0].w, cr[0].ldw, a.S, true, a.A, Hc);
-    u32x4 R[PD][TH];
-    ring_fill(R, fwd_of(cr[0]));
+    Ring<TH> R;
+    ring_fill<TH>(R, fwd_of(cr[0]));
     zero_lds(lds, a.lds);
     __syncthreads();
     row_put16<P>(lds, ss, a.X, 0, a.S, row0, B);
@@ -431,8 +432,8 @@
     row_issue(sh, a.h0, Ha, Ha, row0, B);
     const float m0 = ldg(a.mean0 + min(row0 + (int)(threadIdx.x % TR), B - 1));
     thin_issue(tw, a.fe[3].w, a.fe[3].ldw, Z, true, A, He);
-    u32x4 R[PD][TH];
-    ring_fill(R, bwd_of(a.fe[5], 0));
+    Ring<TH> R;
+    ring_fill<TH>(R, bwd_of(a.fe[5], 0));
     zero_lds(lds, a.lds);
     __syncthreads();
     row_add(d0, d1);
@@ -842,7 +843,7 @@
     g.phase = phase;
     g.qs = q_ws; g.h0s = h0_ws; g.ms = mean_ws;
     const int kd = kd_of(prec);
-    Bump b(1);
+    Bump b;
     g.X = b.r16(TR, ld16(S + A, kd));
     g.CAT = b.r16(TR, ld16(g.Hc + 2 * g.Z, kd));
     g.H1 = b.r16(TR, ld16(g.Hc, kd));
@@ -893,7 +894,7 @@
     g.mse_scale = 2.0f / ((float)B * (float)g.Z);
     g.ld = ld;
     const int w = std::max(g.Z, g.He), kd = kd_of(prec);
-    Bump b(1);
+    Bump b;
     g.X = b.r16(TR, ld16(g.S, kd));
     g.H1 = b.r16(TR, ld16(g.He, kd));
     g.H2 = b.r16(TR, ld16(g.He, kd));
@@ -961,7 +962,7 @@
     }
     g.da = u.da; g.dzsa = u.dzsa; g.ld = ld;
     const int hmax = std::max(g.Ha, std::max(g.He, g.Hc)), kd = kd_of(prec);
-    Bump b(1);
+    Bump b;
     if (phase == 0) {
         g.X = b.r16(TR, ld16(g.S, kd));
         g.CATA = b.r16(TR, ld16(g.Ha + g.Z, kd));
```

New measurement: 18.62 million, median of 6. 1.07x the previous value.
